# kalenforn/clip-based-cross-modal-hash

Hardware: AMD Instinct MI355X
Metric: Hamming query x gallery pairs/sec (fused mAP@all pass, DCMHT COCO-shaped 64-bit) (higher is better)
Workload: dtype u32; 1 GPU; configs[1] DCMHT COCO 64-bit retrieval: Q=5000 queries x R=117218 gallery items per GPU (x1 GPUs, contiguous shards), K=64 bits, C=80 classes, mAP@all; Q=5000, R_per_gpu=117218, K=64, C=80, parallelism=gallery-shard x1, query_blocks=1

## Files before the change

### clip-based-cross-modal-hash_amd/csrc/xmh_scan.hip

```cpp
#include "xmh_common.h"
#include <atomic>
#include <math.h>
#include <mutex>
#include <string.h>
#include <vector>
#include "xmh_scan_bits.h"
#include "xmh_scan_mfma.h"
#include "xmh_scan_kernels.h"

#include <stdlib.h>
#include <type_traits>

namespace {

constexpr int kSlotBudget64 = 9 * 1024;
constexpr int kSlotBudget32 = 5 * 1024;
constexpr int slots_for(int W, bool tern, int counter_bytes) {
    const int nbmax = (tern ? 64 : 32) * W + 1;
    const int budget = counter_bytes == 8 ? kSlotBudget64 : kSlotBudget32;
    const int cap = W > 8 ? 64 : 8;
    int S = 2;
    while (S < cap && nbmax * (64 / S) * counter_bytes > budget) S *= 2;
    return S;
}
inline int instance_words(int W) { return W <= 1 ? 1 : (W <= 2 ? 2 : (W <= 4 ? 4 : (W <= 8 ? 8 : (W <= 16 ? 16 : (W <= 32 ? 32 : 64))))); }
constexpr bool pair_cache_shape(int W, bool tern) { return !tern && (W == 1 || W == 2 || W == 4 || W == 8); }
template <int W, bool TERN>
constexpr bool kPairCacheShape = pair_cache_shape(W, TERN);
constexpr int cache_slots(int W) { return W <= 2 ? 4 : 8; }
static_assert(slots_for(2, false, 4) == 4 && slots_for(2, false, 8) == 4 && slots_for(4, false, 4) == 8 && slots_for(4, false, 8) == 8 &&
              slots_for(8, false, 4) == 8 && slots_for(8, false, 8) == 8, "33..256 bits: the cache geometry is the uncached kernels' own");
constexpr int waves_for(int W, bool tern) { return (W >= 32 && !tern) ? 8 : 1; }
inline size_t aos_ring_bytes(int W, int LW, bool tern) { return (size_t)64 * (((W * (tern ? 2 : 1) + LW) + 3) / 4 * 4) * 4; }

struct WsLayout {
    size_t chunk_hist, below, tot, dpre, cap, tick, gate, ap_part, pair_cache, total;
};

bool r2_selfcheck_ok();
inline bool mfma_env_on() {
    const char* e = getenv("XMH_SCAN_MFMA");
    return !(e && atoi(e) == 0);
}
struct Overrides {
    int mfma = -1;
    bool masked = false;
    bool describe = false;
};
enum class Family { kValu, kR2, kR2w, kBits, kTBits };
Family pass1_family(int K, bool ternary, const Overrides& ov) {
    if (ov.mfma == 0 || !mfma_env_on()) return Family::kValu;
    if (ternary) return K <= 256 ? Family::kTBits : Family::kValu;
    if (K > 128) return K <= 256 ? Family::kBits : Family::kValu;
    if (ov.mfma < 0 && !r2_selfcheck_ok()) return Family::kValu;
    return K <= 64 ? Family::kR2 : Family::kR2w;
}
inline int tbits_tiles(int K) { return K <= 64 ? 2 : (K <= 128 ? 4 : 8); }
inline int ap_r2_mode() {
    const char* e = getenv("XMH_SCAN_AP_R2");
    return e ? (atoi(e) != 0 ? 1 : 0) : 2;
}
constexpr int kAp2Waves = 4, kAp2Groups = 2;
constexpr int kMfmaWaves = 4;
static_assert(xmh::kScanBitsWaves == kMfmaWaves, "k_scan_hist_b takes the plan's query tiles of 64");
constexpr int kBitsMaxChunk = 24192;
struct R2Geom { int nw, nq, blocks_per_cu; int queries() const { return nw * nq * 16; } };
inline R2Geom r2_geom(int K) { return K <= 32 ? R2Geom{4, 4, 1} : (K <= 64 ? R2Geom{4, 4, 2} : R2Geom{4, 2, 2}); }

inline long long cache_cap_mb() {
    const char* cap_env = getenv("XMH_SCAN_CACHE_MB");
    return cap_env ? atoll(cap_env) : 131072;
}
inline bool ap_c_on() {
    const char* e = getenv("XMH_SCAN_AP_C");
    return !(e && atoi(e) == 0);
}
size_t pair_cache_bytes(const xmh_scan_plan& p, int K, bool ternary, Family f) {
    const long long cap_mb = cache_cap_mb();
    const bool tb = f == Family::kTBits;
    if ((ternary && !tb) || K > 256 || cap_mb <= 0 || (!tb && K <= 32 && f != Family::kR2)) return 0;
    if (f == Family::kR2 && ap_r2_mode() == 1) return 0;
    const int S = tb ? 8 : (K <= 64 ? 4 : 8);
    const size_t bytes = (size_t)p.nchunk * (size_t)(p.nqtile * S) * (size_t)((p.chunk + 63) / 64) * (S == 4 ? 1024 : 64 * 4 * xmh::kCache12Dwords);
    return bytes <= (size_t)cap_mb << 20 ? bytes : 0;
}

WsLayout ws_layout(const xmh_scan_plan& p, size_t cache_bytes) {
    WsLayout L;
    const size_t cells = (size_t)p.nchunk * p.nbuckets * p.qpad;
    size_t o = 0;
    auto take = [&](size_t bytes) {
        const size_t at = o;
        o += (bytes + 255) & ~(size_t)255;
        return at;
    };
    L.chunk_hist = take(cells * 4);
    L.below = take(cells * 8);
    L.tot = take((size_t)p.nbuckets * p.qpad * 8);
    L.dpre = take((size_t)p.nbuckets * p.qpad * 8);
    L.cap = take((size_t)p.qpad * 4);
    L.tick = take((size_t)p.nqtile * 4);
    L.gate = take(256 + 8 * 4096);
    L.ap_part = take((size_t)p.nchunk * p.qpad * 4);
    L.pair_cache = take(cache_bytes);
    L.total = o;
    return L;
}

size_t cache_for_workspace(const xmh_scan_plan& p, int K, bool ternary, Family f, size_t ws_bytes) {
    const size_t c = pair_cache_bytes(p, K, ternary, f);
    return c && ws_bytes < ws_layout(p, c).total ? 0 : c;
}

int make_plan(int64_t Q, int64_t R, int K, int ternary, xmh_scan_plan* p, const Overrides& ov = {}) {
    if (Q <= 0 || R <= 0 || K <= 0) return xmh::fail(XMH_EINVAL, "scan plan: bad shape Q=%lld R=%lld K=%d", (long long)Q, (long long)R, K);
    if (R >= (1ll << 24) || Q >= (1ll << 24)) return xmh::fail(XMH_ENOTSUP, "scan plan: shard too large (R=%lld, Q=%lld)", (long long)R, (long long)Q);
    const int64_t nb = ternary ? 2 * (int64_t)K + 1 : (int64_t)K + 1;
    const int Wd = (K + 31) / 32;
    if (Wd > 64 || (ternary && Wd > 8))
        return xmh::fail(XMH_ENOTSUP, "scan plan: K=%d%s (at most 2048 code bits, 256 with zero planes)", K, ternary ? " ternary" : "");
    const int S64 = slots_for(instance_words(Wd), ternary != 0, 8);
    const int64_t lds_ap = nb * (64 / S64) * 8;
    if (lds_ap > 150 * 1024) return xmh::fail(XMH_ENOTSUP, "scan plan: %lld distance buckets need %lld B of LDS per wave; K=%d%s", (long long)nb, (long long)lds_ap, K, ternary ? " ternary" : "");
    const Family fam = pass1_family(K, ternary != 0, ov);
    const bool r2 = fam == Family::kR2 || fam == Family::kR2w;
    int64_t nqt = xmh::ceil_div(Q, 64);
    const int r2q = r2_geom(K).queries();
    if (r2) {
        int64_t l = r2q;
        while (l % 64) l += r2q;
        nqt = xmh::ceil_div(nqt * 64, l) * l / 64;
    }
    const int64_t wpc = 8;
    const int64_t slots = (int64_t)xmh::device_cu_count() * wpc;
    const bool cache_shape = !ternary && K > 32 && K <= 64 && cache_cap_mb() > 0;
    const int64_t rounds = nb <= 33 ? 3 : (nb <= 65 && !cache_shape ? 2 : 1);
    int64_t nchunk = rounds * slots / nqt;
    if (S64 > 8) nchunk = nchunk * 8 / S64;
    const bool mfma = fam != Family::kValu;
    bool fill = false;
    if (mfma) {
        int64_t bsets = nb <= 129 ? 6 : 3;
        if (const char* e = xmh_experiment_env("XMH_BITS_SETS")) bsets = atoi(e) > 0 ? atoi(e) : bsets;
        nchunk = bsets * xmh::device_cu_count() / nqt;
        if (r2) {
            int sets = K > 32 && K <= 64 ? 1 : 2;
            if (const char* e = xmh_experiment_env("XMH_R2_SETS")) sets = atoi(e) > 0 ? atoi(e) : sets;
            nchunk = (int64_t)sets * xmh::device_cu_count() * r2_geom(K).blocks_per_cu / (nqt * 64 / r2q);
            if (const char* e = xmh_experiment_env("XMH_R2_FILL")) fill = atoi(e) != 0 && fam == Family::kR2 && sets == 1 && cache_shape && ap_r2_mode() != 1;
        }
    }
    if (nchunk < 1) nchunk = 1;
    if (nchunk > 8 && !fill) nchunk = (nchunk + 4) / 8 * 8;
    int64_t chunk = xmh::ceil_div(R, nchunk);
    if (chunk < kMinChunk) chunk = kMinChunk;
    if (chunk > kMaxChunk) chunk = kMaxChunk;
    chunk = xmh::ceil_div(chunk, 8) * 8;
    if (mfma) {
        chunk = xmh::ceil_div(chunk, 64) * 64;
        int64_t bits_max = kBitsMaxChunk;
        if (const char* e = xmh_experiment_env("XMH_BITS_MAX_CHUNK")) bits_max = atoll(e) / 64 * 64 > 0 ? atoll(e) / 64 * 64 : bits_max;
        if (!r2 && chunk > bits_max) {
            nchunk = xmh::ceil_div(xmh::ceil_div(R, bits_max), 8) * 8;
            chunk = xmh::ceil_div(xmh::ceil_div(R, nchunk), 64) * 64;
        }
    }
    nchunk = xmh::ceil_div(R, chunk);
    p->chunk = chunk;
    p->nchunk = nchunk;
    p->nqtile = nqt;
    p->qpad = nqt * 64;
    p->nbuckets = nb;
    p->ws_bytes = ws_layout(*p, pair_cache_bytes(*p, K, ternary != 0, fam)).total;
    return XMH_OK;
}

int lane_order_ok(hipStream_t st) {
    static int cached[64];
    static bool have[64];
    static std::mutex mu;
    int dev = 0;
    if (hipGetDevice(&dev) != hipSuccess || dev < 0 || dev >= 64) return 0;
    if (getenv("XMH_SCAN_MASKED") != nullptr) return 0;
    std::lock_guard<std::mutex> lock(mu);
    if (have[dev]) return cached[dev];
    int ok = 0;
    {
        const char* fe = getenv("XMH_SCAN_PROBE_FAULT");
        const int fault = fe && atoi(fe) != 0;
        uint32_t* flag = nullptr;
        float* sink = nullptr;
        if (hipMalloc(&flag, 8) == hipSuccess && hipMalloc(&sink, 256) == hipSuccess) {
            uint32_t h[2] = {0, 1};
            int cus = xmh::device_cu_count();
            if (hipMemsetAsync(flag, 0, 8, st) == hipSuccess) {
                hipLaunchKernelGGL(k_probe_lane_order, dim3(1), dim3(64), 0, st, flag);
                hipLaunchKernelGGL(k_probe_lane_order_load, dim3((unsigned)(cus * 25)), dim3(64), 0, st, flag + 1, fault, sink);
                if (hipGetLastError() == hipSuccess && hipMemcpyAsync(h, flag, 8, hipMemcpyDeviceToHost, st) == hipSuccess && hipStreamSynchronize(st) == hipSuccess)
                    ok = h[0] == 1u && h[1] == 0u;
            }
        }
        if (flag) (void)hipFree(flag);
        if (sink) (void)hipFree(sink);
        if (!ok)
            fprintf(stderr, "xmh: the lane-order probe FAILED on device %d%s: same-address returning LDS adds are not served in lane order here; "
                            "pass 2 runs the masked kernels (about 2x slower, same results).\n", dev, fault ? " (XMH_SCAN_PROBE_FAULT set: forced)" : "");
    }
    cached[dev] = ok;
    have[dev] = true;
    return ok;
}

struct DevBuf {
    void* p = nullptr;
    ~DevBuf() { if (p) (void)hipFree(p); }
    bool alloc(size_t n) { return hipMalloc(&p, n) == hipSuccess; }
    template <typename T> T* as() { return static_cast<T*>(p); }
};

template <bool TERN, typename F>
int dispatch_shape(int W, int LW, F&& f) {
#define XMH_CASE(WW, LL) \
    if (W == WW && LW == LL) return f(std::integral_constant<int, WW>{}, std::integral_constant<int, LL>{});
    XMH_CASE(1, 1) XMH_CASE(1, 2) XMH_CASE(1, 3) XMH_CASE(1, 4)
    XMH_CASE(2, 1) XMH_CASE(2, 2) XMH_CASE(2, 3) XMH_CASE(2, 4)
    XMH_CASE(4, 1) XMH_CASE(4, 2) XMH_CASE(4, 3) XMH_CASE(4, 4)
    XMH_CASE(8, 1) XMH_CASE(8, 2) XMH_CASE(8, 3) XMH_CASE(8, 4)
    if constexpr (!TERN) {
        XMH_CASE(1, 8) XMH_CASE(2, 8) XMH_CASE(4, 8) XMH_CASE(8, 8)
    }
    if constexpr (!TERN) {
        XMH_CASE(16, 1) XMH_CASE(16, 2) XMH_CASE(16, 3) XMH_CASE(16, 4)
        XMH_CASE(32, 1) XMH_CASE(32, 2) XMH_CASE(32, 3) XMH_CASE(32, 4)
        XMH_CASE(64, 1) XMH_CASE(64, 2) XMH_CASE(64, 3) XMH_CASE(64, 4)
    }
#undef XMH_CASE
    return xmh::fail(XMH_ENOTSUP, "scan: unsupported shape W=%d code words (K in {<=32,64,128,256}, binary also 512,1024,2048), Lw=%d label words (C<=128; binary codes up to 256 bits also exactly 8 words: 129..256 classes)%s",
                     W, LW, TERN ? ", ternary" : "");
}

int packed_rank_bits(int K, int64_t R) {
    const char* e = getenv("XMH_SCAN_PACK32");
    if (e && e[0] == '0') return 0;
    if (!(K > 64 || (e && e[0] == 'a'))) return 0;
    const int64_t rank_max = R + 2;
    int rank_bits = 0;
    while ((1ll << rank_bits) < rank_max) ++rank_bits;
    return rank_bits > 24 ? 0 : rank_bits;
}

enum class Mode { kUnsharded, kBaseAll, kTotals, kAllToAll };
struct ScanCall {
    const uint32_t *qbits, *qzero, *qlab, *rbits, *rzero, *rlab;
    int64_t Q, R; int K, C;
    void* ws; size_t ws_bytes;
    bool tern;
};
struct Pass2 {
    Mode mode; int64_t k;
    double* ap_sum; int32_t* cap;
    double* map_out;
    const uint32_t *base_all = nullptr, *base_rel = nullptr, *nrel_total = nullptr;
    const uint32_t* hist_g = nullptr;
    int world = 0, rank = 0;
};
enum class Kern { kHistS, kHistR2, kHistR2w, kHistB, kApS, kApC, kApR2 };
enum Gate : unsigned {
    kBySize = 1,
    kByWrap = 2,
    kByWidth = 4,
};
struct Launch {
    Kern kern = Kern::kHistS;
    int W = 0, LW = 0;
    bool tern = false, cache = false;
    int S = 0, NW = 1;
    int nml = 0;
    int eb = 0; bool half = false;
    bool p32 = false, masked = false;
    unsigned gate = 0;
    bool stand_in = false;
};
struct ScanRoute {
    Launch p1;
    size_t cache_bytes = 0;
    int rank_bits = 0;
    Launch p2[3];
    int n2 = 0;
};

ScanRoute scan_route(const xmh_scan_plan& p, const ScanCall& c, Mode mode, const Overrides& ov, hipStream_t st) {
    ScanRoute r;
    const int K = c.K, C = c.C; const bool tern = c.tern; const int64_t R = c.R;
    const Family fam = pass1_family(K, tern, ov);
    const int W = ov.describe ? instance_words((K + 31) / 32) : (K + 31) / 32, LW = (C + 31) / 32;
    const bool lane_ok = ov.describe || (!ov.masked && lane_order_ok(st));
    r.cache_bytes = cache_for_workspace(p, K, tern, fam, c.ws_bytes);
    const bool cache = r.cache_bytes != 0;
    const bool mfma = fam != Family::kValu && LW <= 4 && lane_ok;
    Launch& h = r.p1;
    h.W = W; h.LW = LW; h.tern = tern; h.cache = cache; h.nml = LW <= 2 ? 1 : 2;
    if (!mfma) {
        h.cache = cache && pair_cache_shape(W, tern);
        h.S = h.cache ? cache_slots(W) : slots_for(W, tern, 4);
        h.NW = h.S == 64 ? waves_for(W, tern) : 1;
    } else if (fam == Family::kBits || fam == Family::kTBits) {
        h.kern = Kern::kHistB;
        h.S = fam == Family::kTBits ? tbits_tiles(K) : 4;
    } else {
        const R2Geom g = r2_geom(K);
        h.kern = fam == Family::kR2 ? Kern::kHistR2 : Kern::kHistR2w;
        h.NW = g.nw; h.S = g.nq;
    }
    const bool sharded = mode != Mode::kUnsharded;
    const bool masked = !lane_ok;
    const int rank_bits = sharded || masked ? 0 : packed_rank_bits(K, R);
    const bool fits_fb = sharded || R <= kFloatBitsMaxItems;
    const bool apc_on = ap_c_on();
    const bool byte128 = cache && mfma && fam == Family::kR2w;
    const bool tb = cache && mfma && fam == Family::kTBits;
    const bool apc = cache && apc_on && (byte128 || (K <= 64 && rank_bits == 0)) && !tern && !masked && (mode != Mode::kBaseAll || byte128) && fits_fb;
    const bool apr2 = !cache && mfma && fam == Family::kR2 && ap_r2_mode() != 0 && !masked && mode != Mode::kBaseAll && rank_bits == 0 && fits_fb;
    const bool apc16 = cache && apc_on && ((K > 128 && K <= 256 && !tern) || tb) && !masked && !sharded && R <= kFloatBitsMaxItems;
    const unsigned size_gate = sharded && (apc || apr2) ? kBySize : 0u;
    r.rank_bits = byte128 && apc ? 0 : rank_bits;
    auto add = [&](Kern kern, unsigned gate) -> Launch& { Launch& l = r.p2[r.n2++]; l.kern = kern; l.gate = gate; return l; };
    if (apc) {
        Launch& l = add(Kern::kApC, size_gate | (byte128 ? kByWrap : 0u));
        l.eb = 8; l.half = byte128; l.S = byte128 ? 8 : 4;
    }
    if (apr2) {
        Launch& l = add(Kern::kApR2, size_gate);
        l.W = W; l.LW = LW; l.nml = h.nml; l.NW = kAp2Waves; l.S = kAp2Groups;
    }
    if (apc16) {
        Launch& l = add(Kern::kApC, kByWidth);
        l.eb = 16; l.S = 8;
    }
    if ((apc || apr2) && !size_gate && !byte128) return r;
    Launch s;
    s.kern = Kern::kApS; s.W = tb ? 8 : W; s.LW = LW; s.tern = tern && !tb; s.masked = masked;
    s.cache = cache && !byte128 && !masked && pair_cache_shape(s.W, s.tern);
    s.stand_in = byte128 && apc;
    s.gate = size_gate | (s.stand_in ? kByWrap : 0u) | (r.rank_bits ? kByWidth : 0u);
    for (const bool p32 : {true, false}) {
        if (p32 ? r.rank_bits == 0 : apc16) continue;
        s.p32 = p32;
        s.S = s.cache ? cache_slots(s.W) : slots_for(s.W, s.tern, p32 ? 4 : 8);
        s.NW = s.S == 64 ? waves_for(s.W, s.tern) : 1;
        r.p2[r.n2++] = s;
    }
    return r;
}

int describe_launch(const Launch& l, char* out, size_t n) {
    static const char* const tf[2] = {"false", "true"};
    auto exists = [&](auto tern_c) { return dispatch_shape<decltype(tern_c)::value>(l.W, l.LW, [](auto, auto) { return (int)XMH_OK; }); };
    switch (l.kern) {
    case Kern::kHistS:
    case Kern::kApS:
        if (const int rc = l.tern ? exists(std::true_type{}) : exists(std::false_type{})) return rc;
        if (l.kern == Kern::kHistS) snprintf(out, n, "k_scan_hist_s<%d, %d, %s, %d, %d, %s>", l.W, l.LW, tf[l.tern], l.S, l.NW, tf[l.cache]);
        else
            snprintf(out, n, "k_scan_ap_s<%d, %d, %s, %s, %d, %s, %s, %d, %s>", l.W, l.cache ? 1 : l.LW, tf[l.tern], tf[!l.cache], l.S, tf[l.p32], tf[l.masked],
                     l.NW, tf[l.cache]);
        break;
    case Kern::kHistR2:
    case Kern::kHistR2w:
        snprintf(out, n, "k_scan_hist_%s<%d, %d, %d, %s>", l.kern == Kern::kHistR2 ? "r2" : "r2w", l.nml, l.NW, l.S, tf[l.cache]);
        break;
    case Kern::kHistB: {
        int nsh, nqt;
        xmh::scan_hist_bits_shape(l.S, l.tern, &nsh, &nqt);
        snprintf(out, n, "k_scan_hist_b<%d, %d, %d, %d, %s, %s>", l.S, kMfmaWaves, nsh, nqt, tf[l.cache], tf[l.tern]);
        break;
    }
    case Kern::kApC: snprintf(out, n, "k_scan_ap_c<false, %d, %s>", l.eb, tf[l.half]); break;
    case Kern::kApR2: snprintf(out, n, "k_scan_ap_r2<%d, %d, %d, false>", l.nml, l.NW, l.S); break;
    }
    return XMH_OK;
}

int check_common(const char* who, const ScanCall& c, const xmh_scan_plan& p) {
    if (!c.qbits || !c.rbits || !c.qlab || !c.rlab || !c.ws) return xmh::fail(XMH_EINVAL, "%s: null pointer", who);
    if ((c.qzero == nullptr) != (c.rzero == nullptr)) return xmh::fail(XMH_EINVAL, "%s: zero masks must be given for both sides or neither", who);
    if (c.C <= 0) return xmh::fail(XMH_EINVAL, "%s: C=%d", who, c.C);
    const size_t need = ws_layout(p, 0).total;
    if (c.ws_bytes < need) return xmh::fail(XMH_EINVAL, "%s: workspace too small (%zu < %zu; %zu with the pair cache)", who, c.ws_bytes, need, (size_t)p.ws_bytes);
    return XMH_OK;
}

ScanArgs make_args(const ScanCall& c, const xmh_scan_plan& p) {
    return ScanArgs{c.qbits, c.qzero, c.qlab, c.rbits, c.rzero, c.rlab, (int)c.Q, (int)c.R, c.K, (int)p.chunk, (int)p.nchunk, (int)p.nqtile, (int)p.qpad,
                    (int)p.nbuckets, nullptr, (int)p.nqtile};
}

MfmaArgs r2_args(const ScanCall& c, const Launch& l, const xmh_scan_plan& p, int nqt) {
    MfmaArgs a{c.qbits, (int)c.Q, (int)c.R, c.K, l.W, (int)p.chunk, (int)p.nchunk, nqt, (int)p.nbuckets, (int)p.qpad};
    a.rbits = c.rbits; a.rlab = c.rlab; a.qlab = c.qlab; a.LW = l.LW;
    return a;
}

struct Geom { unsigned grid, block; size_t lds; int nqt, nrun; };
Geom launch_geom(const Launch& l, const xmh_scan_plan& p, int64_t Q) {
    const size_t nb = (size_t)p.nbuckets;
    const bool ap = l.kern == Kern::kApS || l.kern == Kern::kApC || l.kern == Kern::kApR2;
    Geom g{0, 64u * (unsigned)l.NW, 0, 0};
    if (l.kern == Kern::kHistS || l.kern == Kern::kApS) {
        g.lds = ((nb * (64 / l.S) * (ap && !l.p32 ? 2 : 1) + 3) & ~(size_t)3) * 4 * l.NW + (ap && l.cache ? 0 : aos_ring_bytes(l.W, l.LW, l.tern));
        g.nqt = (int)p.nqtile * l.S / l.NW;
    } else if (l.kern == Kern::kApC) {
        g.lds = nb * (64 / l.S) * 8; g.nqt = (int)p.nqtile * l.S;
    } else if (l.kern == Kern::kHistB) {
        g.nqt = (int)(p.qpad / (16 * kMfmaWaves));
    } else {
        g.lds = (size_t)l.NW * l.S * nb * 16 * (ap ? 8 : 4); g.nqt = (int)(p.qpad / (l.NW * l.S * 16));
    }
    g.nrun = g.nqt;
    if (ap) {
        static const bool all_tiles = xmh_experiment_env("XMH_AP_TILES") && atoi(xmh_experiment_env("XMH_AP_TILES")) == 0;
        if (!all_tiles) g.nrun = (int)xmh::ceil_div(Q, p.qpad / g.nqt);
    }
    g.grid = xmh::scan_grid_blocks(g.nrun, (int)p.nchunk);
    return g;
}

template <typename KernT, typename... Args>
int start(const char* who, const Launch& l, const Geom& g, hipStream_t st, KernT kern, int S, int NW, bool cache, Args... args) {
    if (l.S != S || l.NW != NW || l.cache != cache)
        return xmh::fail(XMH_ENOTSUP, "%s: the route names an instance with S=%d NW=%d cache=%d, the one compiled for W=%d LW=%d has S=%d NW=%d cache=%d", who, l.S,
                         l.NW, (int)l.cache, l.W, l.LW, S, NW, (int)cache);
    if (const int rc = xmh::raise_dynamic_lds(reinterpret_cast<const void*>(kern), g.lds, who)) return rc;
    hipLaunchKernelGGL(kern, dim3(g.grid), dim3(g.block), g.lds, st, args...);
    return XMH_OK;
}

struct ScanCtx {
    const ScanCall& c;
    hipStream_t st;
    xmh_scan_plan p;
    ScanRoute r;
    WsLayout L;
    ScanArgs a;
    uint32_t kcap = 0xffffffffu;
    bool capped = false;
    template <typename T> T* at(size_t off) const { return reinterpret_cast<T*>(static_cast<char*>(c.ws) + off); }
    uint32_t* chunk_hist() const { return at<uint32_t>(L.chunk_hist); }
    const uint2* below() const { return at<uint2>(L.below); }
    uint2* tot() const { return at<uint2>(L.tot); }
    uint2* dpre() const { return at<uint2>(L.dpre); }
    uint32_t* cap_ws() const { return at<uint32_t>(L.cap); }
    float* ap_part() const { return at<float>(L.ap_part); }
    ScanArgs args(const Geom& g, bool cached) const { ScanArgs as = a; as.nqt = g.nqt; as.nrun = g.nrun; as.pair_cache = cached ? pair_cache() : nullptr; return as; }
    uint32_t* gate(int word = 0) const { return at<uint32_t>(L.gate) + word; }
    const uint32_t* gate_if(const Launch& l, unsigned g, int word) const { return (l.gate & g) ? gate(word) : nullptr; }
    uint4* pair_cache() const { return r.cache_bytes ? at<uint4>(L.pair_cache) : nullptr; }
};

int plan_call(const char* who, ScanCtx& x, const Overrides& ov) {
    if (const int rc = make_plan(x.c.Q, x.c.R, x.c.K, x.c.tern, &x.p, ov)) return rc;
    return check_common(who, x.c, x.p);
}
void route_call(ScanCtx& x, Mode mode, const Overrides& ov) {
    x.r = scan_route(x.p, x.c, mode, ov, x.st);
    x.a = make_args(x.c, x.p);
    x.L = ws_layout(x.p, x.r.cache_bytes);
}

int valu_hist(const ScanCtx& x) {
    const Launch& h = x.r.p1;
    const Geom g = launch_geom(h, x.p, x.c.Q);
    const ScanArgs as = x.args(g, h.cache);
    auto go = [&](auto kern, int S, int NW, bool cache) {
        xmh::ProfScope prof("scan_hist", x.st);
        return start("xmh_hamming_hist", h, g, x.st, kern, S, NW, cache, as, x.chunk_hist());
    };
    auto launch = [&](auto tern_c) {
        constexpr bool T = decltype(tern_c)::value;
        return dispatch_shape<T>(h.W, h.LW, [&](auto w, auto l) {
            constexpr int WW = decltype(w)::value, LL = decltype(l)::value;
            if constexpr (kPairCacheShape<WW, T>) {
                if (h.cache) return go(k_scan_hist_s<WW, LL, T, cache_slots(WW), 1, true>, cache_slots(WW), 1, true);
            }
            constexpr int S = slots_for(WW, T, 4);
            constexpr int NW = S == 64 ? waves_for(WW, T) : 1;
            return go(k_scan_hist_s<WW, LL, T, S, NW, false>, S, NW, false);
        });
    };
    return h.tern ? launch(std::true_type{}) : launch(std::false_type{});
}

int mfma_hist(const ScanCtx& x) {
    const Launch& h = x.r.p1;
    const xmh_scan_plan& p = x.p;
    const Geom g = launch_geom(h, p, x.c.Q);
    uint32_t* chunk_hist = x.chunk_hist();
    uint4* cache = x.pair_cache();
    if (h.kern == Kern::kHistB) {
        xmh::ScanBitsArgs a{x.c.rbits, x.c.rlab, x.c.qbits, x.c.qlab, (int)x.c.Q, (int)x.c.R, x.c.K, h.W, h.LW, (int)p.chunk, (int)p.nchunk, g.nqt,
                            (int)p.nbuckets, (int)p.qpad};
        a.rzero = x.c.rzero; a.qzero = x.c.qzero;
        return xmh::launch_scan_hist_bits(a, h.S, chunk_hist, cache, x.st);
    }
    hipLaunchKernelGGL(k_scan_touch, dim3(xmh::scan_grid_blocks(kTouchPerChunk, (int)p.nchunk)), dim3(256), 0, x.st, x.c.rbits, x.c.rlab, x.c.R, h.W, h.LW,
                       p.chunk, (int)p.nchunk, x.at<uint32_t>(x.L.tick), (int)((x.L.gate + 256 - x.L.tick) / 4));
    XMH_LAUNCH_CHECK("xmh_hamming_hist control words");
    const MfmaArgs a = r2_args(x.c, h, p, g.nqt);
    xmh::ProfScope prof("scan_hist", x.st);
    auto go = [&](auto kern, int NW, int NQ, bool cached, auto... wrap_word) { return start("xmh_hamming_hist", h, g, x.st, kern, NQ, NW, cached, a, chunk_hist, cache, wrap_word...); };
    if (h.kern == Kern::kHistR2w) {
        uint32_t* ovf = x.gate(kGateWrapped);
        return h.nml == 1 ? (h.cache ? go(k_scan_hist_r2w<1, 4, 2, true>, 4, 2, true, ovf) : go(k_scan_hist_r2w<1, 4, 2, false>, 4, 2, false, ovf))
                          : (h.cache ? go(k_scan_hist_r2w<2, 4, 2, true>, 4, 2, true, ovf) : go(k_scan_hist_r2w<2, 4, 2, false>, 4, 2, false, ovf));
    }
    return h.nml == 1 ? (h.cache ? go(k_scan_hist_r2<1, 4, 4, true>, 4, 4, true) : go(k_scan_hist_r2<1, 4, 4, false>, 4, 4, false))
                      : (h.cache ? go(k_scan_hist_r2<2, 4, 4, true>, 4, 4, true) : go(k_scan_hist_r2<2, 4, 4, false>, 4, 4, false));
}

int hamming_hist_impl(const ScanCall& c, uint32_t* hist_all, uint32_t* hist_rel, xmh_stream_t stream, const Overrides& ov) {
    ScanCtx x{c, xmh::as_stream(stream)};
    if (const int rc = plan_call("xmh_hamming_hist", x, ov)) return rc;
    route_call(x, Mode::kUnsharded, ov);
    const xmh_scan_plan& p = x.p;
    const Kern kern = x.r.p1.kern;
    if (kern == Kern::kHistS || kern == Kern::kHistB) XMH_HIP(hipMemsetAsync(x.at<char>(x.L.tick), 0, x.L.gate + 256 - x.L.tick, x.st));
    if (const int rc = kern == Kern::kHistS ? valu_hist(x) : mfma_hist(x)) return rc;
    XMH_LAUNCH_CHECK("xmh_hamming_hist");
    hipLaunchKernelGGL(k_scan_below, dim3((unsigned)p.nqtile, (unsigned)xmh::ceil_div(p.nbuckets, 4)), dim3(256), 0, x.st, x.chunk_hist(), (int)p.qpad,
                       (int)p.nbuckets, (int)p.nchunk, kern != Kern::kHistS ? kRelHi16 : 0u, x.at<uint2>(x.L.below), x.tot(), x.at<uint32_t>(x.L.tick), (int)c.Q, x.dpre(),
                       x.cap_ws(), x.gate(), hist_all, hist_rel);
    XMH_LAUNCH_CHECK("xmh_hamming_hist below");
    return XMH_OK;
}

}

extern "C" int xmh_scan_plan_make(int64_t Q, int64_t R, int K, int ternary, xmh_scan_plan* plan_host) {
    if (!plan_host) return xmh::fail(XMH_EINVAL, "xmh_scan_plan_make: null plan");
    return make_plan(Q, R, K, ternary, plan_host);
}

extern "C" size_t xmh_scan_pair_cache_bytes(int64_t Q, int64_t R, int K, int ternary) {
    xmh_scan_plan p;
    if (make_plan(Q, R, K, ternary, &p)) return 0;
    return pair_cache_bytes(p, K, ternary != 0, pass1_family(K, ternary != 0, {}));
}

extern "C" size_t xmh_scan_pair_cache_offset(int64_t Q, int64_t R, int K, int ternary) {
    xmh_scan_plan p;
    if (make_plan(Q, R, K, ternary, &p)) return (size_t)-1;
    return ws_layout(p, 0).pair_cache;
}

extern "C" size_t xmh_scan_ws_bytes_nocache(int64_t Q, int64_t R, int K, int ternary) {
    xmh_scan_plan p;
    if (make_plan(Q, R, K, ternary, &p)) return 0;
    return ws_layout(p, 0).total;
}

extern "C" int xmh_scan_describe(int64_t Q, int64_t R, int K, int C, int ternary, char* out, size_t out_bytes) {
    if (!out || out_bytes < 64) return xmh::fail(XMH_EINVAL, "xmh_scan_describe: buffer too small");
    xmh_scan_plan p;
    if (const int rc = make_plan(Q, R, K, ternary, &p)) return rc;
    Overrides ov;
    ov.describe = true;
    const ScanCall c{nullptr, nullptr, nullptr, nullptr, nullptr, nullptr, Q, R, K, C, nullptr, (size_t)p.ws_bytes, ternary != 0};
    const ScanRoute r = scan_route(p, c, Mode::kUnsharded, ov, nullptr);
    char p1[160], p2[200] = "", one[120];
    if (const int rc = describe_launch(r.p1, p1, sizeof(p1))) return rc;
    for (const bool p32 : {true, false})
        for (int i = 0; i < r.n2; ++i) {
            if (r.p2[i].stand_in || r.p2[i].p32 != p32) continue;
            if (const int rc = describe_launch(r.p2[i], one, sizeof(one))) return rc;
            const size_t at = strlen(p2);
            snprintf(p2 + at, sizeof(p2) - at, "%s%s", at ? "|" : "", one);
        }
    if ((size_t)snprintf(out, out_bytes, "pass1=%s;pass2=%s", p1, p2) >= out_bytes) return xmh::fail(XMH_EINVAL, "xmh_scan_describe: buffer too small");
    return XMH_OK;
}

extern "C" int xmh_hamming_hist(const uint32_t* qbits, const uint32_t* qzero, const uint32_t* qlab,
                                const uint32_t* rbits, const uint32_t* rzero, const uint32_t* rlab, int64_t Q, int64_t R,
                                int K, int C, void* ws, size_t ws_bytes, uint32_t* hist_all, uint32_t* hist_rel,
                                xmh_stream_t stream) {
    XMH_RANGE("xmh_hamming_hist (pass 1)");
    const ScanCall c{qbits, qzero, qlab, rbits, rzero, rlab, Q, R, K, C, ws, ws_bytes, qzero != nullptr};
    return hamming_hist_impl(c, hist_all, hist_rel, stream, {});
}

namespace {
int ap_offsets(const ScanCtx& x, const Pass2& o) {
    const xmh_scan_plan& p = x.p;
    if (o.mode == Mode::kUnsharded) return XMH_OK;
    if (o.mode == Mode::kAllToAll)
        hipLaunchKernelGGL(k_shard_scatter_offsets, dim3((unsigned)xmh::ceil_div(p.qpad, 256), (unsigned)p.nbuckets + 1), dim3(256), 0, x.st,
                           reinterpret_cast<const uint2*>(o.hist_g), (int)p.nbuckets, (int)(p.qpad / o.world), (int)x.c.Q, (int)p.qpad, o.k, x.dpre(), x.cap_ws(),
                           o.cap, x.gate(2));
    else if (o.mode == Mode::kTotals)
        hipLaunchKernelGGL(k_shard_offsets_dpre, dim3((unsigned)p.nqtile), dim3(256), 0, x.st, reinterpret_cast<const uint2*>(o.hist_g), o.world, o.rank,
                           (int)x.c.Q, (int)p.qpad, (int)p.nbuckets, o.k, x.dpre(), x.cap_ws(), o.cap, x.gate(2));
    else
        hipLaunchKernelGGL(k_scan_dpre, dim3((unsigned)p.nqtile), dim3(256), 0, x.st, (const uint2*)x.tot(), (int)x.c.Q, (int)p.qpad, (int)p.nbuckets, o.base_all,
                           o.base_rel, o.nrel_total, o.k, x.dpre(), x.cap_ws(), o.cap, (uint32_t*)nullptr, (uint32_t*)nullptr, (uint32_t*)nullptr, x.gate(2));
    XMH_LAUNCH_CHECK(o.mode == Mode::kAllToAll ? "xmh_hamming_map_sharded_offsets scatter" : (o.mode == Mode::kTotals ? "xmh_hamming_map_sharded offsets" : "xmh_hamming_ap dpre"));
    return XMH_OK;
}

int ap_launch_c(const ScanCtx& x, const Launch& l) {
    const Geom g = launch_geom(l, x.p, x.c.Q);
    const ScanArgs as = x.args(g, true);
    xmh::ProfScope prof("scan_ap", x.st);
    auto go = [&](auto kc, int S) {
        return start("xmh_hamming_ap", l, g, x.st, kc, S, 1, l.cache, as, x.below(), (const uint2*)x.dpre(), (const uint32_t*)x.cap_ws(), x.ap_part(),
                     x.gate_if(l, kBySize, 2), x.kcap, x.gate_if(l, kByWrap, kGateWrapped), x.gate_if(l, kByWidth, 0), l.gate & kByWidth ? x.r.rank_bits : 0);
    };
    if (l.eb == 16) return x.capped ? go(k_scan_ap_c<true, 16>, 8) : go(k_scan_ap_c<false, 16>, 8);
    if (l.half) return x.capped ? go(k_scan_ap_c<true, 8, true>, 8) : go(k_scan_ap_c<false, 8, true>, 8);
    return x.capped ? go(k_scan_ap_c<true, 8>, 4) : go(k_scan_ap_c<false, 8>, 4);
}

int ap_launch_r2(const ScanCtx& x, const Launch& l) {
    const Geom g = launch_geom(l, x.p, x.c.Q);
    const MfmaArgs ma = r2_args(x.c, l, x.p, g.nrun);
    xmh::ProfScope prof("scan_ap", x.st);
    auto go = [&](auto kern) {
        return start("xmh_hamming_ap", l, g, x.st, kern, kAp2Groups, kAp2Waves, l.cache, ma, x.below(), (const uint2*)x.dpre(), (const uint32_t*)x.cap_ws(), x.ap_part(),
                     x.gate_if(l, kBySize, 2), x.kcap);
    };
    return l.nml == 1 ? (x.capped ? go(k_scan_ap_r2<1, kAp2Waves, kAp2Groups, true>) : go(k_scan_ap_r2<1, kAp2Waves, kAp2Groups, false>))
                      : (x.capped ? go(k_scan_ap_r2<2, kAp2Waves, kAp2Groups, true>) : go(k_scan_ap_r2<2, kAp2Waves, kAp2Groups, false>));
}

int ap_launch_s(const ScanCtx& x, const Launch& l) {
    const Geom g = launch_geom(l, x.p, x.c.Q);
    const ScanArgs as = x.args(g, l.cache);
    auto go = [&](auto kern, int S, int NW, bool cache, const uint32_t* run_if) {
        xmh::ProfScope prof(l.p32 ? "scan_ap32" : "scan_ap", x.st);
        return start("xmh_hamming_ap", l, g, x.st, kern, S, NW, cache, as, x.below(), (const uint2*)x.dpre(), (const uint32_t*)x.cap_ws(), x.ap_part(),
                     (const uint32_t*)x.gate(), x.r.rank_bits, x.kcap, x.gate_if(l, kBySize, 2), run_if);
    };
    auto by_shape = [&](auto tern_c, auto cap_c, auto p32_c, auto masked_c) {
        constexpr bool T = decltype(tern_c)::value, CP = decltype(cap_c)::value, P32 = decltype(p32_c)::value, MK = decltype(masked_c)::value;
        return dispatch_shape<T>(l.W, l.LW, [&](auto w, auto lw) {
            constexpr int WW = decltype(w)::value, LL = decltype(lw)::value;
            if constexpr (P32 && MK) return xmh::fail(XMH_ENOTSUP, "xmh_hamming_ap: the masked fallback runs 64-bit counters only");
            else {
                if constexpr (kPairCacheShape<WW, T> && !MK) {
                    if (l.cache)
                        return go(k_scan_ap_s<WW, 1, T, CP, cache_slots(WW), P32, MK, 1, true>, cache_slots(WW), 1, true, nullptr);
                }
                (void)CP;
                constexpr int S = slots_for(WW, T, P32 ? 4 : 8);
                constexpr int NW = S == 64 ? waves_for(WW, T) : 1;
                return go(k_scan_ap_s<WW, LL, T, true, S, P32, MK, NW, false>, S, NW, false, x.gate_if(l, kByWrap, kGateWrapped));
            }
        });
    };
    using T1 = std::true_type; using T0 = std::false_type;
    auto by_mask = [&](auto t, auto c, auto w) { return l.masked ? by_shape(t, c, w, T1{}) : by_shape(t, c, w, T0{}); };
    auto by_width = [&](auto t, auto c) { return l.p32 ? by_mask(t, c, T1{}) : by_mask(t, c, T0{}); };
    auto by_cap = [&](auto t) { return x.capped ? by_width(t, T1{}) : by_width(t, T0{}); };
    return l.tern ? by_cap(T1{}) : by_cap(T0{});
}

int ap_reduce(const ScanCtx& x, const Pass2& o) {
    const int64_t Q = x.c.Q;
    const unsigned nred = (unsigned)xmh::ceil_div(Q, 64);
    if (o.map_out && nred <= 4096) {
        hipLaunchKernelGGL(k_ap_reduce_map, dim3(nred), dim3(256), 0, x.st, (const float*)x.ap_part(), (int)Q, (int)x.p.qpad, (int)x.p.nchunk,
                           (const uint32_t*)x.cap_ws(), x.kcap, o.cap, o.ap_sum, x.at<double>(x.L.gate + 256), x.gate(1), o.map_out);
        XMH_LAUNCH_CHECK("xmh_hamming_map reduce+finalize");
        return XMH_OK;
    }
    hipLaunchKernelGGL(k_ap_reduce, dim3(nred), dim3(256), 0, x.st, (const float*)x.ap_part(), (int)Q, (int)x.p.qpad, (int)x.p.nchunk, o.ap_sum,
                       o.mode != Mode::kUnsharded ? (const uint32_t*)nullptr : (const uint32_t*)x.cap_ws(), x.kcap, o.cap);
    XMH_LAUNCH_CHECK("xmh_hamming_ap reduce");
    if (o.map_out) {
        hipLaunchKernelGGL(k_map_finalize, dim3(1), dim3(256), 0, x.st, (const double*)o.ap_sum, (const int32_t*)o.cap, Q, o.map_out);
        XMH_LAUNCH_CHECK("xmh_hamming_map finalize");
    }
    return XMH_OK;
}

static std::atomic<int> g_verify{0};
constexpr int XMH_EVERIFY_CODE = -74;

int hamming_ap_impl(const ScanCall& c, const Pass2& o, xmh_stream_t stream, const Overrides& ov);

int verify_against_masked(const ScanCall& c, const Pass2& o, xmh_stream_t stream) {
    hipStream_t st = xmh::as_stream(stream);
    const int64_t Q = c.Q;
    std::vector<double> a1((size_t)Q), a0((size_t)Q);
    std::vector<int32_t> c1((size_t)Q), c0((size_t)Q);
    XMH_HIP(hipMemcpyAsync(a1.data(), o.ap_sum, (size_t)Q * 8, hipMemcpyDeviceToHost, st));
    XMH_HIP(hipMemcpyAsync(c1.data(), o.cap, (size_t)Q * 4, hipMemcpyDeviceToHost, st));
    XMH_HIP(hipStreamSynchronize(st));
    Overrides ov;
    ov.mfma = 0;
    ov.masked = true;
    xmh_scan_plan p;
    if (const int rc = make_plan(Q, c.R, c.K, c.tern, &p, ov)) return rc;
    const size_t small = ws_layout(p, 0).total;
    DevBuf ws2, ap2, cap2;
    if (!ws2.alloc(small) || !ap2.alloc((size_t)Q * 8) || !cap2.alloc((size_t)Q * 4))
        return xmh::fail(XMH_ENOMEM, "xmh_scan_verify: no room for the second evaluation (%zu bytes)", small);
    ScanCall again = c; again.ws = ws2.p; again.ws_bytes = small;
    const Pass2 o2{Mode::kUnsharded, o.k, ap2.as<double>(), cap2.as<int32_t>(), nullptr};
    if (const int rc = hamming_hist_impl(again, nullptr, nullptr, stream, ov)) return rc;
    if (const int rc = hamming_ap_impl(again, o2, stream, ov)) return rc;
    XMH_HIP(hipMemcpyAsync(a0.data(), ap2.p, (size_t)Q * 8, hipMemcpyDeviceToHost, st));
    XMH_HIP(hipMemcpyAsync(c0.data(), cap2.p, (size_t)Q * 4, hipMemcpyDeviceToHost, st));
    XMH_HIP(hipStreamSynchronize(st));
    if (const char* fe = getenv("XMH_SCAN_VERIFY_FAULT")) {
        const int64_t at = atoll(fe) % Q;
        a1[(size_t)at] *= 1.0 + 1e-3;
    }
    int64_t bad = -1, nbad = 0;
    for (int64_t i = 0; i < Q; ++i) {
        const bool same = c1[(size_t)i] == c0[(size_t)i] && fabs(a1[(size_t)i] - a0[(size_t)i]) <= 4e-6 * fabs(a0[(size_t)i]) + 1e-9;
        if (!same) { if (bad < 0) bad = i; ++nbad; }
    }
    if (nbad)
        return xmh::fail(XMH_EVERIFY_CODE, "xmh_scan_verify: %lld of %lld queries differ between the lane-order kernels and the masked re-derivation "
                         "(first: query %lld, AP sum %.9g vs %.9g, divisor %d vs %d)", (long long)nbad, (long long)Q, (long long)bad, a1[(size_t)bad], a0[(size_t)bad],
                         c1[(size_t)bad], c0[(size_t)bad]);
    return XMH_OK;
}

int hamming_ap_impl(const ScanCall& c, const Pass2& o, xmh_stream_t stream, const Overrides& ov) {
    ScanCtx x{c, xmh::as_stream(stream)};
    if (const int rc = plan_call("xmh_hamming_ap", x, ov)) return rc;
    if (!o.ap_sum || !o.cap) return xmh::fail(XMH_EINVAL, "xmh_hamming_ap: null output");
    const int ext = (o.base_all != nullptr) + (o.base_rel != nullptr) + (o.nrel_total != nullptr);
    if (ext != 0 && ext != 3) return xmh::fail(XMH_EINVAL, "xmh_hamming_ap: base_all, base_rel and nrel_total go together");
    route_call(x, o.mode, ov);
    x.kcap = o.k > 0 && o.k < (int64_t)0xffffffffll ? (uint32_t)o.k : 0xffffffffu;
    x.capped = o.k > 0;
    if (const int rc = ap_offsets(x, o)) return rc;
    for (int i = 0; i < x.r.n2; ++i) {
        const Launch& l = x.r.p2[i];
        if (const int rc = l.kern == Kern::kApC ? ap_launch_c(x, l) : (l.kern == Kern::kApR2 ? ap_launch_r2(x, l) : ap_launch_s(x, l))) return rc;
        XMH_LAUNCH_CHECK("xmh_hamming_ap");
    }
    if (const int rc = ap_reduce(x, o)) return rc;
    if (g_verify.load(std::memory_order_relaxed) && !ov.masked && o.mode == Mode::kUnsharded) return verify_against_masked(c, o, stream);
    return XMH_OK;
}

bool selfcheck_eval(const ScanCall& c, int force, std::vector<uint32_t>& hist, std::vector<double>& ap, std::vector<int32_t>& cap) {
    Overrides ov;
    ov.mfma = force;
    const int64_t Q = c.Q;
    xmh_scan_plan p;
    if (make_plan(Q, c.R, c.K, 0, &p, ov) != XMH_OK) return false;
    const size_t nb = (size_t)p.nbuckets;
    DevBuf ws, dh, dap, dcap;
    if (!ws.alloc(p.ws_bytes) || !dh.alloc(2 * Q * nb * 4) || !dap.alloc(Q * 8) || !dcap.alloc(Q * 4)) return false;
    ScanCall run = c; run.ws = ws.p; run.ws_bytes = p.ws_bytes;
    const Pass2 o{Mode::kUnsharded, 0, dap.as<double>(), dcap.as<int32_t>(), nullptr};
    uint32_t* h = dh.as<uint32_t>();
    if (hamming_hist_impl(run, h, h + Q * nb, nullptr, ov) != XMH_OK) return false;
    if (hamming_ap_impl(run, o, nullptr, ov) != XMH_OK) return false;
    hist.resize(2 * Q * nb); ap.resize(Q); cap.resize(Q);
    if (hipDeviceSynchronize() != hipSuccess) return false;
    return hipMemcpy(hist.data(), dh.p, hist.size() * 4, hipMemcpyDeviceToHost) == hipSuccess && hipMemcpy(ap.data(), dap.p, Q * 8, hipMemcpyDeviceToHost) == hipSuccess &&
           hipMemcpy(cap.data(), dcap.p, Q * 4, hipMemcpyDeviceToHost) == hipSuccess;
}

bool r2_selfcheck_ok() {
    static int state[64];
    static std::mutex mu;
    int dev = 0;
    if (hipGetDevice(&dev) != hipSuccess || dev < 0 || dev >= 64) return true;
    const char* e = getenv("XMH_SCAN_M2_SELFCHECK");
    if (e && atoi(e) == 0) return true;
    std::lock_guard<std::mutex> lock(mu);
    if (state[dev]) return state[dev] == 1;
    state[dev] = 1;
    const int64_t Q = 200, R = 9000;
    bool same = true, ran = true;
    const int cases[6][2] = {{64, 80}, {40, 80}, {16, 80}, {100, 80}, {64, 128}, {100, 128}};
    for (const auto& kc : cases) {
        const int K = kc[0], C = kc[1], LW = (C + 31) / 32;
        const int W = (K + 31) / 32;
        std::vector<uint32_t> qb(Q * W), ql(Q * LW), rb(R * W), rl(R * LW);
        uint64_t x = 0x9E3779B97F4A7C15ull ^ (uint64_t)K;
        auto rnd = [&]() { x ^= x << 13; x ^= x >> 7; x ^= x << 17; return (uint32_t)(x >> 16); };
        const uint32_t last = K % 32 ? (1u << (K % 32)) - 1 : 0xffffffffu;
        for (auto& v : qb) v = rnd();
        for (int64_t i = 0; i < R; ++i)
            for (int w = 0; w < W; ++w) rb[i * W + w] = (i > 64 && (rnd() & 3) == 0) ? rb[(rnd() % 64) * W + w] : rnd();
        for (int64_t i = 0; i < Q; ++i) qb[i * W + W - 1] &= last;
        for (int64_t i = 0; i < R; ++i) rb[i * W + W - 1] &= last;
        const uint32_t lastl = C % 32 ? (1u << (C % 32)) - 1 : 0xffffffffu;
        for (int64_t i = 0; i < Q * LW; ++i) ql[i] = rnd() & rnd() & rnd() & (i % LW == LW - 1 ? lastl : 0xffffffffu);
        for (int64_t i = 0; i < R * LW; ++i) rl[i] = rnd() & rnd() & rnd() & (i % LW == LW - 1 ? lastl : 0xffffffffu);
        if (C == 80) {
            for (int64_t i = 0; i < Q; ++i) ql[i * LW] |= 1u;
            for (int64_t i = 0; i < R; i += 7) rl[i * LW] |= 1u;
        } else {
            auto one = [&](uint32_t* l, int c) { for (int w = 0; w < LW; ++w) l[w] = 0u; l[c >> 5] = 1u << (c & 31); };
            for (int64_t i = 0; i < Q; i += 2) one(&ql[i * LW], i % 8 == 0 ? (int)(i * 3 % 64) : 64 + (int)(i * 7 % 64));
            for (int64_t i = 0; i < R; ++i) {
                if (i % 3 == 0) one(&rl[i * LW], 64 + (int)(i * 5 % 64));
                else if (i % 3 == 1) for (int w = 0; w < LW; ++w) rl[i * LW + w] = 0u;
            }
            for (int w = 0; w < LW; ++w) ql[1 * LW + w] = rl[2 * LW + w] = rl[5000 * LW + w] = 0xffffffffu;
        }
        std::vector<uint32_t> h1, h0;
        std::vector<double> a1, a0;
        std::vector<int32_t> c1, c0;
        DevBuf dq, dql, dr, drl;
        auto up = [](DevBuf& d, const std::vector<uint32_t>& v) { return d.alloc(v.size() * 4) && hipMemcpy(d.p, v.data(), v.size() * 4, hipMemcpyHostToDevice) == hipSuccess; };
        if (!up(dq, qb) || !up(dql, ql) || !up(dr, rb) || !up(drl, rl)) { ran = false; break; }
        const ScanCall c{dq.as<uint32_t>(), nullptr, dql.as<uint32_t>(), dr.as<uint32_t>(), nullptr, drl.as<uint32_t>(), Q, R, K, C, nullptr, 0, false};
        if (!selfcheck_eval(c, 1, h1, a1, c1) || !selfcheck_eval(c, 0, h0, a0, c0)) { ran = false; break; }
        bool ap_close = true;
        for (int64_t i = 0; i < Q; ++i) ap_close = ap_close && fabs(a1[i] - a0[i]) <= 4e-6 * fabs(a0[i]) + 1e-9;
        if (h1 != h0 || c1 != c0 || !ap_close) { same = false; break; }
    }
    if (e && atoi(e) == 2) same = false;
    if (!ran) {
        state[dev] = 0;
        return true;
    }
    if (!same) {
        state[dev] = 2;
        fprintf(stderr, "xmh: k_scan_hist_r2 self-check FAILED on device %d (results differ from the VALU kernels): falling back to the VALU scan "
                        "for this process.  Please report the hipcc / ROCm versions.\n", dev);
    }
    return state[dev] == 1;
}
}

extern "C" int xmh_scan_verify(int on) {
    g_verify.store(on != 0 ? 1 : 0, std::memory_order_relaxed);
    return XMH_OK;
}

extern "C" int xmh_hamming_ap(const uint32_t* qbits, const uint32_t* qzero, const uint32_t* qlab, const uint32_t* rbits,
                              const uint32_t* rzero, const uint32_t* rlab, int64_t Q, int64_t R, int K, int C, void* ws,
                              size_t ws_bytes, const uint32_t* base_all, const uint32_t* base_rel,
                              const uint32_t* nrel_total, int64_t k, double* ap_sum, int32_t* cap, xmh_stream_t stream) {
    XMH_RANGE("xmh_hamming_ap (pass 2)");
    const ScanCall c{qbits, qzero, qlab, rbits, rzero, rlab, Q, R, K, C, ws, ws_bytes, qzero != nullptr};
    Pass2 o{base_all ? Mode::kBaseAll : Mode::kUnsharded, k, ap_sum, cap, nullptr};
    o.base_all = base_all; o.base_rel = base_rel; o.nrel_total = nrel_total;
    return hamming_ap_impl(c, o, stream, {});
}

extern "C" int xmh_hamming_map(const uint32_t* qbits, const uint32_t* qzero, const uint32_t* qlab, const uint32_t* rbits,
                               const uint32_t* rzero, const uint32_t* rlab, int64_t Q, int64_t R, int K, int C, void* ws,
                               size_t ws_bytes, int64_t k, double* ap_sum, int32_t* cap, double* map_out, xmh_stream_t stream) {
    XMH_RANGE("xmh_hamming_map (pass 2 + mean)");
    if (!map_out) return xmh::fail(XMH_EINVAL, "xmh_hamming_map: null output");
    const ScanCall c{qbits, qzero, qlab, rbits, rzero, rlab, Q, R, K, C, ws, ws_bytes, qzero != nullptr};
    return hamming_ap_impl(c, Pass2{Mode::kUnsharded, k, ap_sum, cap, map_out}, stream, {});
}

extern "C" size_t xmh_scan_totals_offset(int64_t Q, int64_t R, int K, int ternary, size_t* bytes) {
    xmh_scan_plan p;
    if (make_plan(Q, R, K, ternary, &p)) return (size_t)-1;
    if (bytes) *bytes = (size_t)p.nbuckets * p.qpad * 8;
    return ws_layout(p, 0).tot;
}

extern "C" int xmh_hamming_map_sharded(const uint32_t* qbits, const uint32_t* qzero, const uint32_t* qlab, const uint32_t* rbits,
                                       const uint32_t* rzero, const uint32_t* rlab, int64_t Q, int64_t R, int K, int C, void* ws,
                                       size_t ws_bytes, const uint32_t* hist_gathered, int world, int rank, int64_t k, double* ap_sum,
                                       int32_t* cap, double* map_partial, xmh_stream_t stream) {
    XMH_RANGE("xmh_hamming_map_sharded (pass 2)");
    if (!hist_gathered || !map_partial) return xmh::fail(XMH_EINVAL, "xmh_hamming_map_sharded: null pointer");
    if (world <= 0 || rank < 0 || rank >= world) return xmh::fail(XMH_EINVAL, "xmh_hamming_map_sharded: bad world=%d rank=%d", world, rank);
    const ScanCall c{qbits, qzero, qlab, rbits, rzero, rlab, Q, R, K, C, ws, ws_bytes, qzero != nullptr};
    Pass2 o{Mode::kTotals, k, ap_sum, cap, map_partial};
    o.hist_g = hist_gathered; o.world = world; o.rank = rank;
    return hamming_ap_impl(c, o, stream, {});
}

extern "C" int xmh_shard_slice_offsets(const uint32_t* totals_slices, int world, int nbuckets, int slice, uint32_t* offsets_out, xmh_stream_t stream) {
    XMH_RANGE("xmh_shard_slice_offsets");
    if (!totals_slices || !offsets_out) return xmh::fail(XMH_EINVAL, "xmh_shard_slice_offsets: null pointer");
    if (world <= 0 || nbuckets <= 0 || slice <= 0) return xmh::fail(XMH_EINVAL, "xmh_shard_slice_offsets: bad arguments (world=%d nb=%d slice=%d)", world, nbuckets, slice);
    hipLaunchKernelGGL(k_shard_slice_offsets, dim3((unsigned)xmh::ceil_div(slice, 64)), dim3(256), 0, xmh::as_stream(stream),
                       reinterpret_cast<const uint2*>(totals_slices), world, nbuckets, slice, reinterpret_cast<uint2*>(offsets_out));
    XMH_LAUNCH_CHECK("xmh_shard_slice_offsets");
    return XMH_OK;
}

extern "C" int xmh_hamming_map_sharded_offsets(const uint32_t* qbits, const uint32_t* qzero, const uint32_t* qlab, const uint32_t* rbits,
                                               const uint32_t* rzero, const uint32_t* rlab, int64_t Q, int64_t R, int K, int C, void* ws,
                                               size_t ws_bytes, const uint32_t* offsets, int world, int64_t k, double* ap_sum, int32_t* cap,
                                               double* map_partial, xmh_stream_t stream) {
    XMH_RANGE("xmh_hamming_map_sharded_offsets (pass 2)");
    if (!offsets || !map_partial) return xmh::fail(XMH_EINVAL, "xmh_hamming_map_sharded_offsets: null pointer");
    const ScanCall c{qbits, qzero, qlab, rbits, rzero, rlab, Q, R, K, C, ws, ws_bytes, qzero != nullptr};
    xmh_scan_plan p;
    if (const int rc = make_plan(Q, R, K, c.tern, &p)) return rc;
    if (world <= 0 || p.qpad % world) return xmh::fail(XMH_EINVAL, "xmh_hamming_map_sharded_offsets: qpad=%lld is not a multiple of world=%d", (long long)p.qpad, world);
    Pass2 o{Mode::kAllToAll, k, ap_sum, cap, map_partial};
    o.hist_g = offsets; o.world = world;
    return hamming_ap_impl(c, o, stream, {});
}

extern "C" int xmh_map_finalize(const double* ap_sum, const int32_t* cap, int64_t Q, double* map_out, xmh_stream_t stream) {
    XMH_RANGE("xmh_map_finalize");
    if (!ap_sum || !cap || !map_out || Q <= 0) return xmh::fail(XMH_EINVAL, "xmh_map_finalize: bad arguments");
    hipLaunchKernelGGL(k_map_finalize, dim3(1), dim3(256), 0, xmh::as_stream(stream), ap_sum, cap, Q, map_out);
    XMH_LAUNCH_CHECK("xmh_map_finalize");
    return XMH_OK;
}

extern "C" int xmh_shard_offsets(const uint32_t* hist_gathered, int world, int rank, int64_t Q, int nbuckets, uint32_t* base_all,
                                 uint32_t* base_rel, uint32_t* nrel_total, xmh_stream_t stream) {
    XMH_RANGE("xmh_shard_offsets");
    if (!hist_gathered || !base_all || !base_rel || !nrel_total) return xmh::fail(XMH_EINVAL, "xmh_shard_offsets: null pointer");
    if (world <= 0 || rank < 0 || rank >= world || Q <= 0 || nbuckets <= 0 || Q >= (1ll << 24))
        return xmh::fail(XMH_EINVAL, "xmh_shard_offsets: bad arguments (world=%d rank=%d Q=%lld nb=%d)", world, rank, (long long)Q, nbuckets);
    hipLaunchKernelGGL(k_shard_offsets, dim3((unsigned)Q), dim3(64), 0, xmh::as_stream(stream), hist_gathered, world, rank, (int)Q, nbuckets,
                       base_all, base_rel, nrel_total);
    XMH_LAUNCH_CHECK("xmh_shard_offsets");
    return XMH_OK;
}
```

### clip-based-cross-modal-hash_amd/csrc/xmh_scan_mfma.h

```cpp
#pragma once
#include "xmh_common.h"
#include "xmh_scan_map.h"
#include <type_traits>

namespace {

constexpr int kMaxChunk = 32768;
constexpr uint32_t kF23 = 0x4B000000u;
constexpr int64_t kFloatBitsMaxItems = (1ll << 23) - 3;
constexpr int kMinChunk = 256;

struct ScanArgs {
    const uint32_t* qbits;
    const uint32_t* qzero;
    const uint32_t* qlab;
    const uint32_t* rbits;
    const uint32_t* rzero;
    const uint32_t* rlab;
    int Q, R, K;
    int chunk, nchunk, nqt, qpad, nb;
    uint4* pair_cache;
    int nrun;
};

__device__ __forceinline__ bool map_block(const ScanArgs& a, int& chunk_id, int& qtile) {
    return xmh::scan_block_map((int)blockIdx.x, a.nrun, a.nchunk, chunk_id, qtile);
}

typedef int v4i __attribute__((ext_vector_type(4)));

struct MfmaArgs {
    const uint32_t* qbits;
    int Q, R, K, W;
    int chunk, nchunk, nqt, nb, qpad;
    const uint32_t* rbits = nullptr;
    const uint32_t* rlab = nullptr;
    const uint32_t* qlab = nullptr;
    int LW = 0;
};

__device__ __forceinline__ bool map_block(const MfmaArgs& a, int& chunk_id, int& qtile) {
    return xmh::scan_block_map((int)blockIdx.x, a.nqt, a.nchunk, chunk_id, qtile);
}

__device__ __forceinline__ v4i label_query_f4(uint32_t w, uint32_t one) {
    v4i r;
#pragma unroll
    for (int j = 0; j < 4; ++j) r[j] = (int)(((w >> j) & 0x11111111u) * one);
    return r;
}
__device__ __forceinline__ v4i label_item_f4(uint32_t w) {
    return v4i{(int)(w & 0x11111111u), (int)(w & 0x22222222u), (int)(w & 0x44444444u), (int)((w >> 1) & 0x44444444u)};
}

template <int NML, int NW, int NQ, bool CACHE>
__device__ __forceinline__ void scan_hist_r2_body(const MfmaArgs& a, uint32_t* __restrict__ chunk_hist, uint4* __restrict__ pair_cache) {
    static_assert(NML == 1 || NML == 2, "one i8 label tile (at most 64 classes) or one FP4 label tile (65-128 classes)");
    constexpr bool F4 = NML == 2;
    constexpr int NMI = 2, NMQ = 3;
    constexpr bool REGS = true;
    extern __shared__ __attribute__((aligned(16))) uint32_t lds[];
    int chunk_id, qtile;
    if (!map_block(a, chunk_id, qtile)) return;
    const int lane = threadIdx.x & 63, wave = threadIdx.x >> 6;
    const int ql = lane & 15, slot = lane >> 4;
    const int t16 = (qtile * NW + wave) * NQ;
    const int ncell = a.nb * 16;
    uint32_t* cnt = lds + (wave * NQ) * ncell;
    for (int e = lane; e < NQ * ncell; e += 64) cnt[e] = 0u;
    v4i bq[NQ][NMQ], cq[NQ], kqv[REGS ? NQ : 1];
    bool valid[NQ];
    const int rsh = 4 * (slot & 1), rwi = slot >> 1;
#pragma unroll
    for (int h = 0; h < NQ; ++h) {
        valid[h] = (t16 + h) * 16 + ql < a.Q;
        int pcq = 0;
        {
            const int64_t q = (int64_t)(t16 + h) * 16 + ql;
            uint32_t qw = 0u;
            if (valid[h]) {
                for (int w = 0; w < a.W; ++w) pcq += __popc(a.qbits[q * a.W + w]);
                if (rwi < a.W) qw = a.qbits[q * a.W + rwi];
            }
            qw >>= rsh;
#pragma unroll
            for (int j = 0; j < 4; ++j) {
                const uint32_t t = (qw >> j) & 0x01010101u;
                const bool on = valid[h] && rwi < a.W;
                if (j & 1) {
                    bq[h][0][j] = on ? (int)(0x20202020u ^ (t * 0xc0u)) : 0;
                    bq[h][1][j] = on ? (int)(0x01010101u ^ (t * 0xfeu)) : 0;
                } else {
                    bq[h][0][j] = on ? (int)(0x40404040u ^ (t << 7)) : 0;
                    bq[h][1][j] = on ? (int)(0x02020202u ^ (t * 0xfcu)) : 0;
                }
            }
            if constexpr (F4) {
                bq[h][2] = label_query_f4(valid[h] && slot < a.LW ? a.qlab[q * a.LW + slot] : 0u, 0x2u);
            } else {
                uint32_t lw = 0u;
                if (valid[h] && rwi < a.LW) lw = a.qlab[q * a.LW + rwi];
                lw >>= rsh;
#pragma unroll
                for (int j = 0; j < 4; ++j) bq[h][2][j] = (int)((lw >> j) & 0x01010101u);
            }
            const int k2 = 2 * pcq;
            kqv[h] = v4i{k2, k2, k2, k2};
        }
        const int c0 = (int)(uint32_t)(uintptr_t)(__attribute__((address_space(3))) uint32_t*)(cnt + h * ncell) + ql * 4 + (valid[h] ? 64 * pcq : 0);
        cq[h] = v4i{c0, c0, c0, c0};
    }
    v4i lab0 = {0x10000, 0x10000, 0x10000, 0x10000};
    asm volatile("" : "+v"(lab0));
#pragma unroll
    for (int h = 0; h < NQ; ++h) asm volatile("" : "+v"(cq[h]));
#pragma unroll
    for (int h = 0; h < (REGS ? NQ : 1); ++h) asm volatile("" : "+v"(kqv[h]));
    const int64_t lo = (int64_t)chunk_id * a.chunk;
    const int64_t hi = (lo + a.chunk < a.R) ? lo + a.chunk : a.R;
    const int nbat = (int)((hi - lo + 63) >> 6);
    const int64_t bat0 = lo >> 6;
    uint4* crow[NQ];
#pragma unroll
    for (int h = 0; h < NQ; ++h)
        crow[h] = CACHE ? pair_cache + ((int64_t)chunk_id * (a.qpad >> 4) + (t16 + h)) * ((a.chunk + 63) >> 6) * 64 + lane : nullptr;
    uint32_t wcur[4][NMI], wnxt[4][NMI];
    const int ritem = 4 * (lane & 3) + ((lane & 15) >> 2);
    const int wi_c = rwi < a.W ? rwi : a.W - 1;
    const int lwi = F4 ? slot : rwi;
    const int wi_l = lwi < a.LW ? lwi : (a.LW > 0 ? a.LW - 1 : 0);
    auto load_words = [&](int64_t batch, uint32_t (&w)[4][NMI]) {
        const int64_t first = batch * 64;
        if (first + 64 <= (int64_t)a.R) {
            const uint32_t* __restrict__ pc = a.rbits + (first + ritem) * a.W + wi_c;
            const uint32_t* __restrict__ pl = a.rlab + (first + ritem) * a.LW + wi_l;
#pragma unroll
            for (int g = 0; g < 4; ++g) {
                w[g][0] = pc[g * 16 * a.W];
                w[g][1] = pl[g * 16 * a.LW];
            }
        } else {
#pragma unroll
            for (int g = 0; g < 4; ++g) {
                const int64_t item = first + g * 16 + ritem;
                const int64_t it = item < a.R ? item : (int64_t)a.R - 1;
                const uint32_t ok = item < a.R ? 0xffffffffu : 0u;
                w[g][0] = a.rbits[it * a.W + wi_c] & ok;
                w[g][1] = a.rlab[it * a.LW + wi_l] & ok;
            }
        }
    };
    auto build = [&](v4i (&At)[NMI], const uint32_t (&w)[NMI]) {
        const uint32_t xa = w[0] >> rsh, xb = w[0] >> (rsh + 2);
        At[0][0] = (int)(xa & 0x01010101u);
        At[0][1] = (int)(xa & 0x02020202u);
        At[0][2] = (int)(xb & 0x01010101u);
        At[0][3] = (int)(xb & 0x02020202u);
        if constexpr (F4) {
            At[1] = label_item_f4(w[1]);
        } else {
            const uint32_t y = w[1] >> rsh;
#pragma unroll
            for (int j = 0; j < 4; ++j) At[1][j] = (int)(y & (0x01010101u << j));
        }
    };
    load_words(bat0, wcur);
#ifdef XMH_ABL_NOBUILD
    v4i A[4][NMI];
#endif
    for (int i = 0; i < nbat; ++i) {
#ifdef XMH_ABL_NOLOADW
        if (i == 0) load_words(bat0, wnxt);
#else
        load_words(bat0 + (i + 1 < nbat ? i + 1 : i), wnxt);
#endif
#ifndef XMH_ABL_NOBUILD
        v4i A[REGS ? 4 : 2][NMI];
#endif
        uint32_t cw[NQ][4];
        v4i addr_p, d2_p, lab_p;
#ifndef XMH_R2_NOPS
#define XMH_R2_NOPS 0
#endif
#if XMH_R2_NOPS == 0
#define XMH_R2_OPEN "s_nop 3\n\t"
#define XMH_R2_EVAL_CLOSE "s_nop 7"
#define XMH_R2_TAIL "s_nop 7\n\ts_nop 3"
#elif XMH_R2_NOPS == 1
#define XMH_R2_OPEN "s_nop 1\n\t"
#define XMH_R2_EVAL_CLOSE "s_nop 7"
#define XMH_R2_TAIL "s_nop 7\n\ts_nop 3"
#elif XMH_R2_NOPS == 2
#define XMH_R2_OPEN ""
#define XMH_R2_EVAL_CLOSE "s_nop 7"
#define XMH_R2_TAIL "s_nop 7\n\ts_nop 3"
#elif XMH_R2_NOPS == 3
#define XMH_R2_OPEN "s_nop 1\n\t"
#define XMH_R2_EVAL_CLOSE "s_nop 3"
#define XMH_R2_TAIL "s_nop 1"
#else
#define XMH_R2_OPEN ""
#define XMH_R2_EVAL_CLOSE "s_nop 3"
#define XMH_R2_TAIL "s_nop 1"
#endif
#ifdef XMH_ABL_NOMIN
#define XMH_VMIN "; "
#else
#define XMH_VMIN "v_min_u32 "
#endif
#ifdef XMH_ABL_MINFULL
#undef XMH_VMIN
#define XMH_VMIN "v_and_b32 "
#endif
#ifdef XMH_ABL_NOADD
#define XMH_ADD(A, D) "s_nop 0\n\t"
#else
#define XMH_ADD(A, D) "ds_add_u32 " A ", " D "\n\t"
#endif
#ifdef XMH_ABL_NOMFMA
#define XMH_MFMA(D, A, B, C) "s_nop 0\n\t"
#define XMH_MFMA_F4(D, A, B, C) "s_nop 0\n\t"
#else
#define XMH_MFMA(D, A, B, C) "v_mfma_i32_16x16x64_i8 " D ", " A ", " B ", " C "\n\t"
#define XMH_MFMA_F4(D, A, B, C) "v_mfma_f32_16x16x128_f8f6f4 " D ", " A ", " B ", " C " cbsz:4 blgp:4\n\t"
#endif
#define XMH_SDWA(J) "dst_sel:BYTE_" #J " dst_unused:UNUSED_PRESERVE src0_sel:BYTE_0 src1_sel:BYTE_0\n\t"
#define XMH_R2_FUSED_CACHE(LAB)                                                                                                                   \
    asm volatile(XMH_R2_OPEN LAB("%0", "%8", "%9", "%10")                                                                                         \
                 XMH_VMIN "%4, 0x10001, %24\n\t" XMH_VMIN "%5, 0x10001, %25\n\t" XMH_VMIN "%6, 0x10001, %26\n\t" XMH_VMIN "%7, 0x10001, %27\n\t" \
                 "v_or_b32_sdwa %3, %16, %4 dst_sel:BYTE_0 dst_unused:UNUSED_PAD src0_sel:BYTE_0 src1_sel:BYTE_0\n\t"                            \
                 XMH_ADD("%20", "%4")                                                                                                             \
                 XMH_MFMA("%1", "%11", "%12", "%13")                                                                                              \
                 "v_or_b32_sdwa %3, %17, %5 " XMH_SDWA(1) XMH_ADD("%21", "%5") "v_or_b32_sdwa %3, %18, %6 " XMH_SDWA(2)                           \
                 XMH_MFMA("%2", "%11", "%14", "%15")                                                                                              \
                 XMH_ADD("%22", "%6") "v_or_b32_sdwa %3, %19, %7 " XMH_SDWA(3) XMH_ADD("%23", "%7")                                               \
                 : "=&v"(lab), "=&v"(addr), "=&v"(d2), "=&v"(w), "=&v"(i0), "=&v"(i1), "=&v"(i2), "=&v"(i3)                                        \
                 : "v"(At[1]), "v"(bq[h][2]), "v"(lab0), "v"(At[0]), "v"(bq[h][0]), "v"(cq[h]), "v"(bq[h][1]), "v"(kqv[REGS ? h : 0]),             \
                   "v"(d2_p[0]), "v"(d2_p[1]), "v"(d2_p[2]), "v"(d2_p[3]), "v"(addr_p[0]), "v"(addr_p[1]), "v"(addr_p[2]), "v"(addr_p[3]),         \
                   "v"(lab_p[0]), "v"(lab_p[1]), "v"(lab_p[2]), "v"(lab_p[3])                                                                      \
                 : "memory")
#define XMH_R2_FUSED_PLAIN(LAB)                                                                                                                   \
    asm volatile(XMH_R2_OPEN LAB("%0", "%6", "%7", "%8")                                                                                          \
                 XMH_VMIN "%2, 0x10001, %16\n\t" XMH_VMIN "%3, 0x10001, %17\n\t" XMH_VMIN "%4, 0x10001, %18\n\t" XMH_VMIN "%5, 0x10001, %19\n\t" \
                 XMH_MFMA("%1", "%9", "%10", "%11")                                                                                               \
                 XMH_ADD("%12", "%2") XMH_ADD("%13", "%3") XMH_ADD("%14", "%4") XMH_ADD("%15", "%5")                                              \
                 : "=&v"(lab), "=&v"(addr), "=&v"(i0), "=&v"(i1), "=&v"(i2), "=&v"(i3)                                                             \
                 : "v"(At[1]), "v"(bq[h][2]), "v"(lab0), "v"(At[0]), "v"(bq[h][0]), "v"(cq[h]),                                                    \
                   "v"(addr_p[0]), "v"(addr_p[1]), "v"(addr_p[2]), "v"(addr_p[3]), "v"(lab_p[0]), "v"(lab_p[1]), "v"(lab_p[2]), "v"(lab_p[3])      \
                 : "memory")
#define XMH_R2_EVAL_CACHE(LAB)                                                                                                                    \
    asm volatile(XMH_R2_OPEN LAB("%0", "%3", "%4", "%5") XMH_MFMA("%1", "%6", "%7", "%8") XMH_MFMA("%2", "%6", "%9", "%10") XMH_R2_EVAL_CLOSE     \
                 : "=&v"(lab), "=&v"(addr), "=&v"(d2)                                                                                             \
                 : "v"(At[1]), "v"(bq[h][2]), "v"(lab0), "v"(At[0]), "v"(bq[h][0]), "v"(cq[h]), "v"(bq[h][1]), "v"(kqv[REGS ? h : 0]))
#define XMH_R2_EVAL_PLAIN(LAB)                                                                                                                    \
    asm volatile(XMH_R2_OPEN LAB("%0", "%2", "%3", "%4") XMH_MFMA("%1", "%5", "%6", "%7") XMH_R2_EVAL_CLOSE                                       \
                 : "=&v"(lab), "=&v"(addr)                                                                                                        \
                 : "v"(At[1]), "v"(bq[h][2]), "v"(lab0), "v"(At[0]), "v"(bq[h][0]), "v"(cq[h]))
        auto fused = [&](const v4i (&At)[NMI], int h, v4i& addr, v4i& d2, v4i& lab, uint32_t& w) {
            uint32_t i0, i1, i2, i3;
            if constexpr (F4 && CACHE) XMH_R2_FUSED_CACHE(XMH_MFMA_F4);
            else if constexpr (F4) XMH_R2_FUSED_PLAIN(XMH_MFMA_F4);
            else if constexpr (CACHE) XMH_R2_FUSED_CACHE(XMH_MFMA);
            else XMH_R2_FUSED_PLAIN(XMH_MFMA);
        };
        auto evaluate = [&](const v4i (&At)[NMI], int h, v4i& addr, v4i& d2, v4i& lab) {
            if constexpr (F4 && CACHE) XMH_R2_EVAL_CACHE(XMH_MFMA_F4);
            else if constexpr (F4) XMH_R2_EVAL_PLAIN(XMH_MFMA_F4);
            else if constexpr (CACHE) XMH_R2_EVAL_CACHE(XMH_MFMA);
            else XMH_R2_EVAL_PLAIN(XMH_MFMA);
        };
        auto consume = [&](uint32_t& w, const v4i (&live)[NMI]) {
            uint32_t i0, i1, i2, i3;
            if (CACHE) {
                asm volatile(
                    XMH_VMIN "%1, 0x10001, %5\n\t" XMH_VMIN "%2, 0x10001, %6\n\t" XMH_VMIN "%3, 0x10001, %7\n\t" XMH_VMIN "%4, 0x10001, %8\n\t"
                    "v_or_b32_sdwa %0, %9, %1 dst_sel:BYTE_0 dst_unused:UNUSED_PAD src0_sel:BYTE_0 src1_sel:BYTE_0\n\t"
                    XMH_ADD("%13", "%1")
                    "v_or_b32_sdwa %0, %10, %2 " XMH_SDWA(1) XMH_ADD("%14", "%2") "v_or_b32_sdwa %0, %11, %3 " XMH_SDWA(2)
                    XMH_ADD("%15", "%3") "v_or_b32_sdwa %0, %12, %4 " XMH_SDWA(3) XMH_ADD("%16", "%4")
                    : "=&v"(w), "=&v"(i0), "=&v"(i1), "=&v"(i2), "=&v"(i3)
                    : "v"(lab_p[0]), "v"(lab_p[1]), "v"(lab_p[2]), "v"(lab_p[3]), "v"(d2_p[0]), "v"(d2_p[1]), "v"(d2_p[2]), "v"(d2_p[3]), "v"(addr_p[0]),
                      "v"(addr_p[1]), "v"(addr_p[2]), "v"(addr_p[3]), "v"(live[0]), "v"(live[1]), "v"(live[NMI - 1])
                    : "memory");
            } else {
                asm volatile(
                    XMH_VMIN "%0, 0x10001, %4\n\t" XMH_VMIN "%1, 0x10001, %5\n\t" XMH_VMIN "%2, 0x10001, %6\n\t" XMH_VMIN "%3, 0x10001, %7\n\t"
                    XMH_ADD("%8", "%0") XMH_ADD("%9", "%1") XMH_ADD("%10", "%2") XMH_ADD("%11", "%3")
                    : "=&v"(i0), "=&v"(i1), "=&v"(i2), "=&v"(i3)
                    : "v"(lab_p[0]), "v"(lab_p[1]), "v"(lab_p[2]), "v"(lab_p[3]), "v"(addr_p[0]), "v"(addr_p[1]), "v"(addr_p[2]), "v"(addr_p[3]), "v"(live[0]),
                      "v"(live[1]), "v"(live[NMI - 1])
                    : "memory");
            }
        };
#undef XMH_R2_EVAL_PLAIN
#undef XMH_R2_EVAL_CACHE
#undef XMH_R2_FUSED_PLAIN
#undef XMH_R2_FUSED_CACHE
#undef XMH_SDWA
#undef XMH_ADD
#undef XMH_MFMA_F4
#undef XMH_MFMA
        auto group = [&](auto gc) {
            constexpr int G = decltype(gc)::value;
            constexpr int SET = REGS ? G : (G & 1);
#pragma unroll
            for (int h = 0; h < NQ; ++h) {
                v4i addr, d2, lab;
                if (G == 0 && h == 0) evaluate(A[SET], h, addr, d2, lab);
                else fused(A[SET], h, addr, d2, lab, cw[(h + NQ - 1) % NQ][h == 0 ? G - 1 : G]);
                addr_p = addr; d2_p = d2; lab_p = lab;
                if (REGS && G > 0 && h == 0) {
                    if constexpr (NMI == 2) asm volatile("" ::"v"(A[REGS ? G - 1 : 0][0]), "v"(A[REGS ? G - 1 : 0][1]));
                    else asm volatile("" ::"v"(A[REGS ? G - 1 : 0][0]), "v"(A[REGS ? G - 1 : 0][1]), "v"(A[REGS ? G - 1 : 0][NMI - 1]));
                }
            }
        };
#ifdef XMH_ABL_NOBUILD
        if (i == 0) {
#endif
        build(A[0], wcur[0]);
        build(A[1], wcur[1]);
        build(A[2], wcur[2]);
        build(A[3], wcur[3]);
#ifdef XMH_ABL_NOBUILD
        }
#endif
        group(std::integral_constant<int, 0>{});
        group(std::integral_constant<int, 1>{});
        group(std::integral_constant<int, 2>{});
        group(std::integral_constant<int, 3>{});
        asm volatile(XMH_R2_TAIL ::: "memory");
        consume(cw[NQ - 1][3], A[3]);
#ifdef XMH_ABL_NOSTORE
        if (CACHE && a.Q < 0) {
#else
        if (CACHE) {
#endif
#pragma unroll
            for (int h = 0; h < NQ; ++h) {
                uint4* dst = crow[h] + (int64_t)i * 64;
                __builtin_nontemporal_store(cw[h][0], &dst->x);
                __builtin_nontemporal_store(cw[h][1], &dst->y);
                __builtin_nontemporal_store(cw[h][2], &dst->z);
                __builtin_nontemporal_store(cw[h][3], &dst->w);
            }
        }
#pragma unroll
        for (int g = 0; g < 4; ++g)
#pragma unroll
            for (int m = 0; m < NMI; ++m) wcur[g][m] = wnxt[g][m];
    }
    const int npad = nbat * 64 - (int)(hi - lo);
    asm volatile("s_waitcnt lgkmcnt(0)" ::: "memory");
    if (npad > 0 && slot == 0) {
#pragma unroll
        for (int h = 0; h < NQ; ++h) {
            if (!valid[h]) continue;
            const int64_t q = (int64_t)(t16 + h) * 16 + ql;
            int dpad = 0;
            for (int w = 0; w < a.W; ++w) dpad += __popc(a.qbits[q * a.W + w]);
            cnt[h * ncell + dpad * 16 + ql] -= (uint32_t)npad << 16;
        }
    }
#pragma unroll
    for (int h = 0; h < NQ; ++h) {
        uint32_t* __restrict__ out = chunk_hist + ((int64_t)chunk_id * a.nb) * a.qpad + (t16 + h) * 16;
        for (int e = lane; e < ncell; e += 64) out[(int64_t)(e >> 4) * a.qpad + (e & 15)] = cnt[h * ncell + e];
    }
}

constexpr int kTouchPerChunk = 8;
__global__ __launch_bounds__(256) void k_scan_touch(const uint32_t* __restrict__ rbits, const uint32_t* __restrict__ rlab, int64_t R, int W, int LW, int64_t chunk,
                                                    int nchunk, uint32_t* __restrict__ ctl, int ctl_words) {
    if (blockIdx.x == 0)
        for (int e = threadIdx.x; e < ctl_words; e += 256) ctl[e] = 0u;
    int c, sub;
    if (!xmh::scan_block_map((int)blockIdx.x, kTouchPerChunk, nchunk, c, sub)) return;
    const int parts = c < (nchunk & ~7) ? kTouchPerChunk : 1;
    if (parts == 1) sub = 0;
    const int64_t lo = (int64_t)c * chunk, hi = lo + chunk < R ? lo + chunk : R;
    uint32_t acc = 0u;
    auto sweep = [&](const uint32_t* base, int64_t w0, int64_t w1) {
        for (int64_t w = w0 + ((int64_t)sub * 256 + threadIdx.x) * 32; w < w1; w += (int64_t)parts * 256 * 32) acc ^= base[w];
    };
    sweep(rbits, lo * W, hi * W);
    sweep(rlab, lo * LW, hi * LW);
    asm volatile("" ::"v"(acc));
}

#ifndef XMH_R2_ATTR
#define XMH_R2_ATTR
#endif
template <int NML, int NW, int NQ, bool CACHE>
__global__ __launch_bounds__(64 * NW) XMH_R2_ATTR void k_scan_hist_r2(MfmaArgs a, uint32_t* __restrict__ chunk_hist, uint4* __restrict__ pair_cache) {
    scan_hist_r2_body<NML, NW, NQ, CACHE>(a, chunk_hist, pair_cache);
}

#define XMH_W_MFMA(D, A, B, C) "v_mfma_i32_16x16x64_i8 %[" D "], %[" A "], %[" B "], %[" C "]\n\t"
#define XMH_W_MFMA_F4(D, A, B, C) "v_mfma_f32_16x16x128_f8f6f4 %[" D "], %[" A "], %[" B "], %[" C "] cbsz:4 blgp:4\n\t"
#define XMH_W_MIN(I, L) "v_min_u32 %[" I "], 0x10001, %[" L "]\n\t"
#define XMH_W_ADD(A, D) "ds_add_u32 %[" A "], %[" D "]\n\t"
#define XMH_W_FUSED_CACHE(LAB) \
    asm volatile("s_nop 3\n\t" LAB("lab", "al0", "bl0", "lab0") XMH_W_MIN("i0", "lp0") XMH_W_MIN("i1", "lp1") XMH_W_MIN("i2", "lp2")                \
                 XMH_W_MIN("i3", "lp3") XMH_W_ADD("ap0", "i0") XMH_W_MFMA("addr", "a0", "ba0", "cq") XMH_W_ADD("ap1", "i1")                         \
                 XMH_W_MFMA("addr", "a1", "ba1", "addr") XMH_W_ADD("ap2", "i2") XMH_W_MFMA("d2", "a0", "bd0", "kq") XMH_W_ADD("ap3", "i3")          \
                 XMH_W_MFMA("d2", "a1", "bd1", "d2")                                                                                                \
                 : [lab] "=&v"(lab), [addr] "=&v"(addr), [d2] "=&v"(d2), [i0] "=&v"(i0), [i1] "=&v"(i1), [i2] "=&v"(i2), [i3] "=&v"(i3)             \
                 : [a0] "v"(At[0]), [a1] "v"(At[1]), [al0] "v"(At[2]), [ba0] "v"(bA[h][0]), [ba1] "v"(bA[h][1]), [bd0] "v"(bD[h][0]),               \
                   [bd1] "v"(bD[h][1]), [bl0] "v"(bL[h]), [lab0] "v"(lab0), [cq] "v"(cq[h]), [kq] "v"(kq[h]), [lp0] "v"(lab_p[0]),                  \
                   [lp1] "v"(lab_p[1]), [lp2] "v"(lab_p[2]), [lp3] "v"(lab_p[3]), [ap0] "v"(addr_p[0]), [ap1] "v"(addr_p[1]), [ap2] "v"(addr_p[2]), \
                   [ap3] "v"(addr_p[3])                                                                                                             \
                 : "memory")
#define XMH_W_FUSED_PLAIN(LAB) \
    asm volatile("s_nop 3\n\t" LAB("lab", "al0", "bl0", "lab0") XMH_W_MIN("i0", "lp0") XMH_W_MIN("i1", "lp1") XMH_W_MIN("i2", "lp2")                 \
                 XMH_W_MIN("i3", "lp3") XMH_W_ADD("ap0", "i0") XMH_W_ADD("ap1", "i1") XMH_W_MFMA("addr", "a0", "ba0", "cq") XMH_W_ADD("ap2", "i2")   \
                 XMH_W_ADD("ap3", "i3") XMH_W_MFMA("addr", "a1", "ba1", "addr")                                                                      \
                 : [lab] "=&v"(lab), [addr] "=&v"(addr), [i0] "=&v"(i0), [i1] "=&v"(i1), [i2] "=&v"(i2), [i3] "=&v"(i3)                              \
                 : [a0] "v"(At[0]), [a1] "v"(At[1]), [al0] "v"(At[2]), [ba0] "v"(bA[h][0]), [ba1] "v"(bA[h][1]), [bl0] "v"(bL[h]), [lab0] "v"(lab0), \
                   [cq] "v"(cq[h]), [lp0] "v"(lab_p[0]), [lp1] "v"(lab_p[1]), [lp2] "v"(lab_p[2]), [lp3] "v"(lab_p[3]), [ap0] "v"(addr_p[0]),        \
                   [ap1] "v"(addr_p[1]), [ap2] "v"(addr_p[2]), [ap3] "v"(addr_p[3])                                                                  \
                 : "memory")
template <int NML, int NW, int NQ, bool CACHE>
__global__ __launch_bounds__(64 * NW) void k_scan_hist_r2w(MfmaArgs a, uint32_t* __restrict__ chunk_hist, uint4* __restrict__ pair_cache,
                                                           uint32_t* __restrict__ ovf) {
    static_assert(NML == 1 || NML == 2, "one i8 label tile (at most 64 classes) or one FP4 label tile (65-128 classes)");
    constexpr bool F4 = NML == 2;
    constexpr int NMC = 2, NMI = NMC + 1;
    extern __shared__ __attribute__((aligned(16))) uint32_t lds[];
    int chunk_id, qtile;
    if (!map_block(a, chunk_id, qtile)) return;
    const int lane = threadIdx.x & 63, wave = threadIdx.x >> 6;
    const int ql = lane & 15, slot = lane >> 4;
    const int t16 = (qtile * NW + wave) * NQ;
    const int ncell = a.nb * 16;
    uint32_t* cnt = lds + (wave * NQ) * ncell;
    for (int e = lane; e < NQ * ncell; e += 64) cnt[e] = 0u;
    const int rsh = 4 * (slot & 1), rwi = slot >> 1;
    v4i bA[NQ][NMC], bD[NQ][NMC], bL[NQ], cq[NQ], kq[NQ];
    bool valid[NQ];
#pragma unroll
    for (int h = 0; h < NQ; ++h) {
        const int64_t q = (int64_t)(t16 + h) * 16 + ql;
        valid[h] = q < a.Q;
        int pcq = 0;
        if (valid[h])
            for (int w = 0; w < a.W; ++w) pcq += __popc(a.qbits[q * a.W + w]);
#pragma unroll
        for (int c = 0; c < NMC; ++c) {
            const int wi = 2 * c + rwi;
            const bool on = valid[h] && wi < a.W;
            const uint32_t qw = (on ? a.qbits[q * a.W + wi] : 0u) >> rsh;
#pragma unroll
            for (int j = 0; j < 4; ++j) {
                const uint32_t t = (qw >> j) & 0x01010101u;
                if (j & 1) {
                    bA[h][c][j] = on ? (int)(0x20202020u ^ (t * 0xc0u)) : 0;
                    bD[h][c][j] = on ? (int)(0x01010101u ^ (t * 0xfeu)) : 0;
                } else {
                    bA[h][c][j] = on ? (int)(0x40404040u ^ (t << 7)) : 0;
                    bD[h][c][j] = on ? (int)(0x02020202u ^ (t * 0xfcu)) : 0;
                }
            }
        }
        if constexpr (F4) {
            bL[h] = label_query_f4(valid[h] && slot < a.LW ? a.qlab[q * a.LW + slot] : 0u, 0x2u);
        } else {
            uint32_t lw = 0u;
            if (valid[h] && rwi < a.LW) lw = a.qlab[q * a.LW + rwi];
            lw >>= rsh;
#pragma unroll
            for (int j = 0; j < 4; ++j) bL[h][j] = (int)((lw >> j) & 0x01010101u);
        }
        const int c0 = (int)(uint32_t)(uintptr_t)(__attribute__((address_space(3))) uint32_t*)(cnt + h * ncell) + ql * 4 + (valid[h] ? 64 * pcq : 0);
        const int k2 = valid[h] ? 2 * pcq : 0;
        cq[h] = v4i{c0, c0, c0, c0};
        kq[h] = v4i{k2, k2, k2, k2};
    }
    v4i lab0 = {0x10000, 0x10000, 0x10000, 0x10000};
    asm volatile("" : "+v"(lab0));
#pragma unroll
    for (int h = 0; h < NQ; ++h) asm volatile("" : "+v"(cq[h]), "+v"(kq[h]));
    const int64_t lo = (int64_t)chunk_id * a.chunk;
    const int64_t hi = (lo + a.chunk < a.R) ? lo + a.chunk : a.R;
    const int nbat = (int)((hi - lo + 63) >> 6);
    const int64_t bat0 = lo >> 6;
    uint4* crow[NQ];
#pragma unroll
    for (int h = 0; h < NQ; ++h)
        crow[h] = CACHE ? pair_cache + ((int64_t)chunk_id * (a.qpad >> 4) + (t16 + h)) * ((a.chunk + 63) >> 6) * 64 + lane : nullptr;
    uint32_t wcur[4][NMI], wnxt[4][NMI];
    const int ritem = 4 * (lane & 3) + ((lane & 15) >> 2);
    int wi_c[NMC];
#pragma unroll
    for (int c = 0; c < NMC; ++c) wi_c[c] = 2 * c + rwi < a.W ? 2 * c + rwi : a.W - 1;
    const int lwi = F4 ? slot : rwi;
    const int wi_l = lwi < a.LW ? lwi : (a.LW > 0 ? a.LW - 1 : 0);
    auto load_words = [&](int64_t batch, uint32_t (&w)[4][NMI]) {
        const int64_t first = batch * 64;
        if (first + 64 <= (int64_t)a.R) {
            const uint32_t* __restrict__ pc = a.rbits + (first + ritem) * a.W;
            const uint32_t* __restrict__ pl = a.rlab + (first + ritem) * a.LW;
#pragma unroll
            for (int g = 0; g < 4; ++g) {
#pragma unroll
                for (int c = 0; c < NMC; ++c) w[g][c] = pc[g * 16 * a.W + wi_c[c]];
                w[g][NMC] = pl[g * 16 * a.LW + wi_l];
            }
        } else {
#pragma unroll
            for (int g = 0; g < 4; ++g) {
                const int64_t item = first + g * 16 + ritem;
                const int64_t it = item < a.R ? item : (int64_t)a.R - 1;
                const uint32_t ok = item < a.R ? 0xffffffffu : 0u;
#pragma unroll
                for (int c = 0; c < NMC; ++c) w[g][c] = a.rbits[it * a.W + wi_c[c]] & ok;
                w[g][NMC] = a.rlab[it * a.LW + wi_l] & ok;
            }
        }
    };
    auto build = [&](v4i (&At)[NMI], const uint32_t (&w)[NMI]) {
#pragma unroll
        for (int c = 0; c < NMC; ++c) {
            const uint32_t xa = w[c] >> rsh, xb = w[c] >> (rsh + 2);
            At[c][0] = (int)(xa & 0x01010101u);
            At[c][1] = (int)(xa & 0x02020202u);
            At[c][2] = (int)(xb & 0x01010101u);
            At[c][3] = (int)(xb & 0x02020202u);
        }
        if constexpr (F4) {
            At[NMC] = label_item_f4(w[NMC]);
        } else {
            const uint32_t y = w[NMC] >> rsh;
#pragma unroll
            for (int j = 0; j < 4; ++j) At[NMC][j] = (int)(y & (0x01010101u << j));
        }
    };
    uint32_t dmax = 0u;
    load_words(bat0, wcur);
    for (int i = 0; i < nbat; ++i) {
        load_words(bat0 + (i + 1 < nbat ? i + 1 : i), wnxt);
        v4i A[4][NMI];
        uint32_t cw[NQ][4];
        v4i addr_p = {0, 0, 0, 0}, d2_p = {0, 0, 0, 0}, lab_p = {0, 0, 0, 0};
        auto fused = [&](const v4i (&At)[NMI], int h, v4i& addr, v4i& d2, v4i& lab, uint32_t& i0, uint32_t& i1, uint32_t& i2, uint32_t& i3) {
            if constexpr (F4 && CACHE) XMH_W_FUSED_CACHE(XMH_W_MFMA_F4);
            else if constexpr (F4) XMH_W_FUSED_PLAIN(XMH_W_MFMA_F4);
            else if constexpr (CACHE) XMH_W_FUSED_CACHE(XMH_W_MFMA);
            else XMH_W_FUSED_PLAIN(XMH_W_MFMA);
        };
        auto pack = [&](uint32_t& w, const v4i& d, uint32_t i0, uint32_t i1, uint32_t i2, uint32_t i3) {
            uint32_t wb;
            asm volatile("v_or_b32_sdwa %[wa], %[d0], %[i0] dst_sel:BYTE_0 dst_unused:UNUSED_PAD src0_sel:BYTE_0 src1_sel:BYTE_0\n\t"
                         "v_or_b32_sdwa %[wb], %[d1], %[i1] dst_sel:BYTE_1 dst_unused:UNUSED_PAD src0_sel:BYTE_0 src1_sel:BYTE_0\n\t"
                         "v_max3_u32 %[mx], %[d0], %[d1], %[mx]\n\t"
                         "v_or_b32_sdwa %[wa], %[d2], %[i2] dst_sel:BYTE_2 dst_unused:UNUSED_PRESERVE src0_sel:BYTE_0 src1_sel:BYTE_0\n\t"
                         "v_or_b32_sdwa %[wb], %[d3], %[i3] dst_sel:BYTE_3 dst_unused:UNUSED_PRESERVE src0_sel:BYTE_0 src1_sel:BYTE_0\n\t"
                         "v_max3_u32 %[mx], %[d2], %[d3], %[mx]\n\t"
                         "v_or_b32 %[wa], %[wa], %[wb]"
                         : [wa] "=&v"(w), [wb] "=&v"(wb), [mx] "+v"(dmax)
                         : [d0] "v"(d[0]), [d1] "v"(d[1]), [d2] "v"(d[2]), [d3] "v"(d[3]), [i0] "v"(i0), [i1] "v"(i1), [i2] "v"(i2), [i3] "v"(i3));
        };
        auto evaluate = [&](const v4i (&At)[NMI], int h, v4i& addr, v4i& d2, v4i& lab) {
            if constexpr (F4) {
                asm volatile("s_nop 3\n\t" XMH_W_MFMA_F4("lab", "al0", "bl0", "lab0") : [lab] "=&v"(lab) : [al0] "v"(At[2]), [bl0] "v"(bL[h]), [lab0] "v"(lab0));
            } else {
                asm volatile("s_nop 3\n\t" XMH_W_MFMA("lab", "al0", "bl0", "lab0") : [lab] "=&v"(lab) : [al0] "v"(At[2]), [bl0] "v"(bL[h]), [lab0] "v"(lab0));
            }
            if (CACHE) {
                asm volatile("s_nop 3\n\t" XMH_W_MFMA("addr", "a0", "ba0", "cq") XMH_W_MFMA("addr", "a1", "ba1", "addr") XMH_W_MFMA("d2", "a0", "bd0", "kq")
                             XMH_W_MFMA("d2", "a1", "bd1", "d2") "s_nop 7"
                             : [addr] "=&v"(addr), [d2] "=&v"(d2)
                             : [a0] "v"(At[0]), [a1] "v"(At[1]), [ba0] "v"(bA[h][0]), [ba1] "v"(bA[h][1]), [bd0] "v"(bD[h][0]), [bd1] "v"(bD[h][1]), [cq] "v"(cq[h]),
                               [kq] "v"(kq[h]));
            } else {
                asm volatile("s_nop 3\n\t" XMH_W_MFMA("addr", "a0", "ba0", "cq") XMH_W_MFMA("addr", "a1", "ba1", "addr") "s_nop 7"
                             : [addr] "=&v"(addr)
                             : [a0] "v"(At[0]), [a1] "v"(At[1]), [ba0] "v"(bA[h][0]), [ba1] "v"(bA[h][1]), [cq] "v"(cq[h]));
            }
        };
        auto consume = [&](uint32_t& i0, uint32_t& i1, uint32_t& i2, uint32_t& i3, const v4i (&live)[NMI]) {
            asm volatile(XMH_W_MIN("i0", "lp0") XMH_W_MIN("i1", "lp1") XMH_W_MIN("i2", "lp2") XMH_W_MIN("i3", "lp3") XMH_W_ADD("ap0", "i0")
                         XMH_W_ADD("ap1", "i1") XMH_W_ADD("ap2", "i2") XMH_W_ADD("ap3", "i3")
                         : [i0] "=&v"(i0), [i1] "=&v"(i1), [i2] "=&v"(i2), [i3] "=&v"(i3)
                         : [lp0] "v"(lab_p[0]), [lp1] "v"(lab_p[1]), [lp2] "v"(lab_p[2]), [lp3] "v"(lab_p[3]), [ap0] "v"(addr_p[0]), [ap1] "v"(addr_p[1]),
                           [ap2] "v"(addr_p[2]), [ap3] "v"(addr_p[3]), "v"(live[0]), "v"(live[1]), "v"(live[2])
                         : "memory");
        };
        auto group = [&](auto gc) {
            constexpr int G = decltype(gc)::value;
#pragma unroll
            for (int h = 0; h < NQ; ++h) {
                v4i addr, d2 = d2_p, lab;
                if (G == 0 && h == 0) {
                    evaluate(A[G], h, addr, d2, lab);
                } else {
                    uint32_t i0, i1, i2, i3;
                    fused(A[G], h, addr, d2, lab, i0, i1, i2, i3);
                    if (CACHE) pack(cw[(h + NQ - 1) % NQ][h == 0 ? G - 1 : G], d2_p, i0, i1, i2, i3);
                }
                addr_p = addr; d2_p = d2; lab_p = lab;
                if (G > 0 && h == 0) {
                    asm volatile("" ::"v"(A[G > 0 ? G - 1 : 0][0]), "v"(A[G > 0 ? G - 1 : 0][1]), "v"(A[G > 0 ? G - 1 : 0][2]));
                }
            }
        };
        build(A[0], wcur[0]);
        build(A[1], wcur[1]);
        build(A[2], wcur[2]);
        build(A[3], wcur[3]);
        group(std::integral_constant<int, 0>{});
        group(std::integral_constant<int, 1>{});
        group(std::integral_constant<int, 2>{});
        group(std::integral_constant<int, 3>{});
        asm volatile("s_nop 7\n\ts_nop 3" ::: "memory");
        {
            uint32_t i0, i1, i2, i3;
            consume(i0, i1, i2, i3, A[3]);
            if (CACHE) pack(cw[NQ - 1][3], d2_p, i0, i1, i2, i3);
        }
#ifdef XMH_ABL_NOSTORE
        if (CACHE && a.Q < 0) {
#else
        if (CACHE) {
#endif
#pragma unroll
            for (int h = 0; h < NQ; ++h) {
                uint4* dst = crow[h] + (int64_t)i * 64;
                __builtin_nontemporal_store(cw[h][0], &dst->x);
                __builtin_nontemporal_store(cw[h][1], &dst->y);
                __builtin_nontemporal_store(cw[h][2], &dst->z);
                __builtin_nontemporal_store(cw[h][3], &dst->w);
            }
        }
#pragma unroll
        for (int g = 0; g < 4; ++g)
#pragma unroll
            for (int m = 0; m < NMI; ++m) wcur[g][m] = wnxt[g][m];
    }
    const int npad = nbat * 64 - (int)(hi - lo);
    asm volatile("s_waitcnt lgkmcnt(0)" ::: "memory");
    if (npad > 0 && slot == 0) {
#pragma unroll
        for (int h = 0; h < NQ; ++h) {
            if (!valid[h]) continue;
            const int64_t q = (int64_t)(t16 + h) * 16 + ql;
            int dpad = 0;
            for (int w = 0; w < a.W; ++w) dpad += __popc(a.qbits[q * a.W + w]);
            cnt[h * ncell + dpad * 16 + ql] -= (uint32_t)npad << 16;
        }
    }
#pragma unroll
    for (int h = 0; h < NQ; ++h) {
        uint32_t* __restrict__ out = chunk_hist + ((int64_t)chunk_id * a.nb) * a.qpad + (t16 + h) * 16;
        for (int e = lane; e < ncell; e += 64) out[(int64_t)(e >> 4) * a.qpad + (e & 15)] = cnt[h * ncell + e];
    }
    if (CACHE && dmax >= 256u) *ovf = 1u;
}
#undef XMH_W_FUSED_PLAIN
#undef XMH_W_FUSED_CACHE
#undef XMH_W_MFMA_F4
#undef XMH_W_MFMA
#undef XMH_W_MIN
#undef XMH_W_ADD

template <bool CAPPED, int EB, bool HALF = false>
__global__ __launch_bounds__(64) void k_scan_ap_c(ScanArgs a, const uint2* __restrict__ below, const uint2* __restrict__ dpre,
                                                  const uint32_t* __restrict__ cap_ws, float* __restrict__ ap_part,
                                                  const uint32_t* __restrict__ items_total, uint32_t kcap, const uint32_t* __restrict__ skip_if = nullptr,
                                                  const uint32_t* __restrict__ nrel_max = nullptr, int rank_bits = 0) {
    static_assert(!HALF || EB == 8, "the 8 x 8 geometry on one-byte entries");
    constexpr int QW = HALF ? 8 : 128 / EB, LOG_QW = QW == 16 ? 4 : 3, S = 64 / QW, EPW = HALF ? 2 : 32 / EB;
    extern __shared__ __attribute__((aligned(16))) uint32_t lds[];
    int chunk_id, qtile;
    if (!map_block(a, chunk_id, qtile)) return;
    if (items_total && (int64_t)*items_total > kFloatBitsMaxItems) return;
    if (skip_if && *skip_if != 0u) return;
    if (nrel_max && rank_bits > 0 && (uint64_t)(*nrel_max) + 2 < (1ull << (32 - rank_bits))) return;
    const int lane = threadIdx.x & 63;
    const int ql = lane & (QW - 1), slot = lane >> LOG_QW;
    const int q0 = qtile * QW, q = q0 + ql;
    const int ncell = a.nb * QW;
    unsigned long long* cnt = reinterpret_cast<unsigned long long*>(lds);
    {
        const uint2* __restrict__ pb = below + ((int64_t)chunk_id * a.nb) * a.qpad + q0;
        const uint2* __restrict__ pd = dpre + q0;
        auto pack = [](uint2 x, uint2 y) {
            return (unsigned long long)(kF23 + x.x + y.x + 1u) | ((unsigned long long)(kF23 + (0x7fffffu - (x.y + y.y + 1u))) << 32);
        };
        int e = lane;
        for (; e + 7 * 64 < ncell; e += 8 * 64) {
            uint2 x[8], y[8];
#pragma unroll
            for (int j = 0; j < 8; ++j) {
                const int ee = e + j * 64;
                const int64_t at = (int64_t)(ee >> LOG_QW) * a.qpad + (ee & (QW - 1));
                x[j] = pb[at];
                y[j] = pd[at];
            }
#pragma unroll
            for (int j = 0; j < 8; ++j) cnt[e + j * 64] = pack(x[j], y[j]);
        }
        for (; e < ncell; e += 64) {
            const int64_t at = (int64_t)(e >> LOG_QW) * a.qpad + (e & (QW - 1));
            cnt[e] = pack(pb[at], pd[at]);
        }
    }
    const uint32_t cntbase = (uint32_t)(uintptr_t)(__attribute__((address_space(3))) uint32_t*)lds + ql * 8;
    const float capf = CAPPED ? (float)min(cap_ws[q], kcap) : 0.0f;
    const int64_t lo = (int64_t)chunk_id * a.chunk;
    const int64_t hi = (lo + a.chunk < a.R) ? lo + a.chunk : a.R;
    float acc = 0.0f;
    auto credit = [&](unsigned long long old, uint32_t m) {
        const float rank = __uint_as_float((uint32_t)old) - 8388608.0f;
        const float ord = 16777215.0f - __uint_as_float((uint32_t)(old >> 32));
        if (CAPPED) m = ord <= capf ? m : 0u;
#ifdef XMH_ABL_AP_NORCP
        acc = fmaf(ord, __uint_as_float(__float_as_uint(rank) & m), acc);
#else
        acc = fmaf(ord, __uint_as_float(__float_as_uint(__builtin_amdgcn_rcpf(rank)) & m), acc);
#endif
    };
    const uint32_t hoff = HALF ? 8u * (uint32_t)(slot >> 2) : 0u;
    const uint32_t hb0 = hoff, hb1 = hoff + 16u, hd0 = hoff + 1u, hd1 = hoff + 17u;
    auto issue1 = [&](uint32_t w, int j, unsigned long long& old, uint32_t& m) {
        uint32_t d;
        if (HALF) {
            m = (uint32_t)__builtin_amdgcn_sbfe((int)w, j ? hb1 : hb0, 1);
            d = __builtin_amdgcn_ubfe(w, j ? hd1 : hd0, EB - 1);
        } else if (EB == 16) {
            m = (uint32_t)__builtin_amdgcn_sbfe((int)w, j, 1);
            d = __builtin_amdgcn_ubfe(w, j + 1, 11);
        } else {
            m = (uint32_t)__builtin_amdgcn_sbfe((int)w, EB * j, 1);
            d = __builtin_amdgcn_ubfe(w, EB * j + 1, EB - 1);
        }
        uint32_t addr;
        if (QW == 16) asm("v_lshl_add_u32 %0, %1, 7, %2" : "=v"(addr) : "v"(d), "v"(cntbase));
        else asm("v_lshl_add_u32 %0, %1, 6, %2" : "=v"(addr) : "v"(d), "v"(cntbase));
        const unsigned long long inc = 1ull | ((unsigned long long)m << 32);
#ifdef XMH_ABL_AP_NOATOMIC
        old = ((unsigned long long)addr << 3) | inc;
        asm volatile("" : "+v"(old));
#else
        asm volatile("ds_add_rtn_u64 %0, %1, %2" : "=v"(old) : "v"(addr), "v"(inc) : "memory");
#endif
    };
    unsigned long long oldA[8], oldB[8];
    uint32_t mA[8], mB[8];
    constexpr bool kFourBatchIterations = true;
    auto issue = [&](unsigned long long (&old)[8], uint32_t (&m)[8], uint32_t wa, uint32_t wb, uint32_t wc, uint32_t wd) {
        if constexpr (EB == 16) {
            const uint32_t sx = __builtin_amdgcn_alignbit(wb, wa, 24), sy = __builtin_amdgcn_alignbit(wc, wb, 28);
#pragma unroll
            for (int u = 0; u < 8; ++u) issue1(XMH_CACHE12_WORD(u, wa, wb, wc, sx, sy), XMH_CACHE12_BIT(u), old[u], m[u]);
        } else {
#pragma unroll
            for (int u = 0; u < 8; ++u) {
                const int wi = u / EPW;
                issue1(wi == 0 ? wa : (wi == 1 ? wb : (wi == 2 ? wc : wd)), u % EPW, old[u], m[u]);
            }
        }
    };
    auto drain8 = [&](unsigned long long (&old)[8], uint32_t (&m)[8]) {
        asm volatile("s_waitcnt lgkmcnt(8)" : "+v"(old[0]), "+v"(old[1]), "+v"(old[2]), "+v"(old[3]), "+v"(old[4]), "+v"(old[5]), "+v"(old[6]), "+v"(old[7])::"memory");
#pragma unroll
        for (int u = 0; u < 8; ++u) credit(old[u], m[u]);
    };
    auto drain0 = [&](unsigned long long (&old)[8], uint32_t (&m)[8]) {
        asm volatile("s_waitcnt lgkmcnt(0)" : "+v"(old[0]), "+v"(old[1]), "+v"(old[2]), "+v"(old[3]), "+v"(old[4]), "+v"(old[5]), "+v"(old[6]), "+v"(old[7])::"memory");
#pragma unroll
        for (int u = 0; u < 8; ++u) credit(old[u], m[u]);
    };
    const int nbatch = (a.chunk + 63) >> 6;
    const uint4* crow = HALF ? a.pair_cache + ((int64_t)chunk_id * (a.nqt >> 1) + (qtile >> 1)) * nbatch * 64 + (slot & 3) * 16 + (qtile & 1) * 8 + ql
                             : a.pair_cache + ((int64_t)chunk_id * a.nqt + qtile) * nbatch * 64 + lane;
    const int nfull = (int)((hi - lo) >> 6);
    asm volatile("s_waitcnt lgkmcnt(0)" ::: "memory");
    const uint32_t* crow12 = reinterpret_cast<const uint32_t*>(a.pair_cache) + (((int64_t)chunk_id * a.nqt + qtile) * nbatch * 64 + lane) * xmh::kCache12Dwords;
    auto cache_words = [&](int64_t batch) -> uint4 {
        if constexpr (EB == 16) {
            typedef uint32_t u32x3_t __attribute__((ext_vector_type(3)));
            const u32x3_t v = __builtin_nontemporal_load(reinterpret_cast<const u32x3_t*>(crow12 + batch * 64 * xmh::kCache12Dwords));
            return make_uint4(v.x, v.y, v.z, 0u);
        } else {
#ifdef XMH_ABL_AP_PLAIN
            return crow[batch * 64];
#else
            typedef uint32_t u32x4_t __attribute__((ext_vector_type(4)));
            const u32x4_t v = __builtin_nontemporal_load(reinterpret_cast<const u32x4_t*>(crow + batch * 64));
            return make_uint4(v.x, v.y, v.z, v.w);
#endif
        }
    };
    uint4 cw = cache_words(0);
    uint4 nw = cache_words(1 < nbatch ? 1 : 0);
    auto next_words = [&](int bi) {
#ifdef XMH_ABL_AP_NOLOAD
        const uint4 nw2 = make_uint4(0x10203040u + bi + lane, 0x18283848u ^ lane, 0x11223344u + 3 * lane, 0x21314151u + bi);
#else
        const uint4 nw2 = cache_words(bi + 2 < nbatch ? bi + 2 : nbatch - 1);
#endif
        return nw2;
    };
    auto slow_batch = [&](const uint4& w4, int count) {
        const uint32_t sx = EB == 16 ? __builtin_amdgcn_alignbit(w4.y, w4.x, 24) : 0u, sy = EB == 16 ? __builtin_amdgcn_alignbit(w4.z, w4.y, 28) : 0u;
#pragma unroll
        for (int t = 0; t < QW; ++t) {
            if (t * S + slot < count) {
                const uint32_t w = EB == 16 ? XMH_CACHE12_WORD(t, w4.x, w4.y, w4.z, sx, sy) : (t < EPW ? w4.x : (t < 2 * EPW ? w4.y : (t < 3 * EPW ? w4.z : w4.w)));
                const uint32_t bit = EB == 16 ? (uint32_t)XMH_CACHE12_BIT(t) : (HALF ? hoff + 16u * (t % EPW) : (uint32_t)(EB * (t % EPW)));
                const uint32_t m = (uint32_t)__builtin_amdgcn_sbfe((int)w, bit, 1), d = __builtin_amdgcn_ubfe(w, bit + 1u, EB == 16 ? 11 : EB - 1);
                const unsigned long long o = atomicAdd(&cnt[d * QW + ql], 1ull | ((unsigned long long)m << 32));
                credit(o, m);
            }
        }
    };
    if (EB == 8 && !HALF) {
        int bi = 0;
        if (kFourBatchIterations) {
            for (; bi + 3 < nfull; bi += 4) {
                const uint4 n0 = next_words(bi);
                issue(oldA, mA, cw.x, cw.y, 0u, 0u);
                issue(oldB, mB, cw.z, cw.w, 0u, 0u);
                drain8(oldA, mA);
                cw = nw;
                nw = n0;
#pragma unroll
                for (int t = 1; t < 4; ++t) {
                    const uint4 nt = next_words(bi + t);
                    issue(oldA, mA, cw.x, cw.y, 0u, 0u);
                    drain8(oldB, mB);
                    issue(oldB, mB, cw.z, cw.w, 0u, 0u);
                    drain8(oldA, mA);
                    cw = nw;
                    nw = nt;
                }
                drain0(oldB, mB);
            }
        }
        for (; bi + 1 < nfull; bi += 2) {
            const uint4 nw2 = next_words(bi);
            issue(oldA, mA, cw.x, cw.y, 0u, 0u);
            issue(oldB, mB, cw.z, cw.w, 0u, 0u);
            drain8(oldA, mA);
            cw = nw;
            nw = nw2;
            const uint4 nw3 = next_words(bi + 1);
            issue(oldA, mA, cw.x, cw.y, 0u, 0u);
            drain8(oldB, mB);
            issue(oldB, mB, cw.z, cw.w, 0u, 0u);
            drain8(oldA, mA);
            drain0(oldB, mB);
            cw = nw;
            nw = nw3;
        }
        if (bi < nfull) {
            const uint4 nw2 = next_words(bi);
            issue(oldA, mA, cw.x, cw.y, 0u, 0u);
            issue(oldB, mB, cw.z, cw.w, 0u, 0u);
            drain8(oldA, mA);
            drain0(oldB, mB);
            cw = nw;
            nw = nw2;
        }
    } else {
        auto words_at = [&](int b) { return cache_words(b < nbatch ? b : nbatch - 1); };
        auto issue4 = [&](unsigned long long (&old)[8], uint32_t (&m)[8], const uint4& r) { issue(old, m, r.x, r.y, r.z, r.w); };
        uint4 r0 = cw, r1 = nw, r2 = words_at(2), r3 = words_at(3);
        int bi = 0;
        for (; bi + 3 < nfull; bi += 4) {
            issue4(oldA, mA, r0);
            r0 = words_at(bi + 4);
            issue4(oldB, mB, r1);
            r1 = words_at(bi + 5);
            drain8(oldA, mA);
            issue4(oldA, mA, r2);
            r2 = words_at(bi + 6);
            drain8(oldB, mB);
            issue4(oldB, mB, r3);
            r3 = words_at(bi + 7);
            drain8(oldA, mA);
            drain0(oldB, mB);
        }
        const int rem = nfull - bi;
        if (rem >= 2) {
            issue4(oldA, mA, r0);
            issue4(oldB, mB, r1);
            drain8(oldA, mA);
            drain0(oldB, mB);
            if (rem == 3) {
                issue4(oldA, mA, r2);
                drain0(oldA, mA);
            }
        } else if (rem == 1) {
            issue4(oldA, mA, r0);
            drain0(oldA, mA);
        }
        cw = rem == 0 ? r0 : (rem == 1 ? r1 : (rem == 2 ? r2 : r3));
    }
    const int cntb = (int)(hi - lo) - nfull * 64;
    slow_batch(cw, cntb);
#pragma unroll
    for (int o = QW; o < 64; o <<= 1) acc += __shfl_xor(acc, o, 64);
    if (slot == 0) ap_part[(int64_t)chunk_id * a.qpad + q] = acc;
}

#define XMH_AP2_SETA "v113", "v115", "v117", "v119", "v[112:113]", "v[114:115]", "v[116:117]", "v[118:119]"
#define XMH_AP2_SETB "v121", "v123", "v125", "v127", "v[120:121]", "v[122:123]", "v[124:125]", "v[126:127]"
#define XMH_AP2_MFMA(D, A, B, C) "v_mfma_i32_16x16x64_i8 %[" D "], %[" A "], %[" B "], " C "\n\t"
#define XMH_AP2_MFMA_F4(D, A, B, C) "v_mfma_f32_16x16x128_f8f6f4 %[" D "], %[" A "], %[" B "], " C " cbsz:4 blgp:4\n\t"
#define XMH_AP2_MAX(H, L) "v_max_i32 " H ", -1, %[" L "]\n\t"
#define XMH_AP2_ADD(O, A, P) "ds_add_rtn_u64 %[" O "], %[" A "], " P "\n\t"
#define XMH_AP2_FUSED_(LAB, H0, H1, H2, H3, P0, P1, P2, P3)                                                                              \
    "s_nop 3\n\t" LAB("lab", "a1", "q1", "0") XMH_AP2_MAX(H0, "l0") XMH_AP2_MAX(H1, "l1") XMH_AP2_MAX(H2, "l2") XMH_AP2_MAX(H3, "l3")    \
    XMH_AP2_MFMA("addr", "a0", "q0", "%[c0]") XMH_AP2_ADD("o0", "p0", P0) XMH_AP2_ADD("o1", "p1", P1) XMH_AP2_ADD("o2", "p2", P2)       \
    XMH_AP2_ADD("o3", "p3", P3)
#define XMH_AP2_TAIL_(H0, H1, H2, H3, P0, P1, P2, P3)                                                                                     \
    XMH_AP2_MAX(H0, "l0") XMH_AP2_MAX(H1, "l1") XMH_AP2_MAX(H2, "l2") XMH_AP2_MAX(H3, "l3") XMH_AP2_ADD("o0", "p0", P0)                   \
    XMH_AP2_ADD("o1", "p1", P1) XMH_AP2_ADD("o2", "p2", P2) XMH_AP2_ADD("o3", "p3", P3)
#define XMH_AP2_FUSED(...) XMH_AP2_FUSED_(__VA_ARGS__)
#define XMH_AP2_TAIL(...) XMH_AP2_TAIL_(__VA_ARGS__)
template <int NML, int NW, int NQ, bool CAPPED>
__global__ __launch_bounds__(64 * NW) void k_scan_ap_r2(MfmaArgs a, const uint2* __restrict__ below, const uint2* __restrict__ dpre,
                                                        const uint32_t* __restrict__ cap_ws, float* __restrict__ ap_part,
                                                        const uint32_t* __restrict__ items_total, uint32_t kcap) {
    using u64 = unsigned long long;
    static_assert(NML == 1 || NML == 2, "one i8 label tile (at most 64 classes) or one FP4 label tile (65-128 classes)");
    constexpr bool F4 = NML == 2;
    constexpr int NMI = 2;
    extern __shared__ __attribute__((aligned(16))) uint32_t lds[];
    int chunk_id, qtile;
    if (!map_block(a, chunk_id, qtile)) return;
    if (items_total && (int64_t)*items_total > kFloatBitsMaxItems) return;
    const int lane = threadIdx.x & 63, wave = threadIdx.x >> 6;
    const int ql = lane & 15, slot = lane >> 4;
    const int t16 = (qtile * NW + wave) * NQ;
    const int ncell = a.nb * 16;
    u64* cnt = reinterpret_cast<u64*>(lds) + (wave * NQ) * ncell;
    auto pack = [](uint2 x, uint2 y) {
        return (u64)(kF23 + x.x + y.x + 1u) | ((u64)(kF23 + (0x7fffffu - (x.y + y.y + 1u))) << 32);
    };
#pragma unroll
    for (int h = 0; h < NQ; ++h) {
        const uint2* __restrict__ pb = below + ((int64_t)chunk_id * a.nb) * a.qpad + (t16 + h) * 16;
        const uint2* __restrict__ pd = dpre + (t16 + h) * 16;
        u64* c = cnt + h * ncell;
        auto cell = [&](int e) { return e; };
        int e = lane;
        for (; e + 3 * 64 < ncell; e += 4 * 64) {
            uint2 x[4], y[4];
#pragma unroll
            for (int j = 0; j < 4; ++j) {
                const int ee = e + j * 64;
                const int64_t at = (int64_t)(ee >> 4) * a.qpad + (ee & 15);
                x[j] = pb[at];
                y[j] = pd[at];
            }
#pragma unroll
            for (int j = 0; j < 4; ++j) c[cell(e + j * 64)] = pack(x[j], y[j]);
        }
        for (; e < ncell; e += 64) {
            const int64_t at = (int64_t)(e >> 4) * a.qpad + (e & 15);
            c[cell(e)] = pack(pb[at], pd[at]);
        }
    }
    v4i bq[NQ], bl[NQ], cq[NQ];
    float capf[NQ], acc[NQ];
    const int rsh = 4 * (slot & 1), rwi = slot >> 1;
#pragma unroll
    for (int h = 0; h < NQ; ++h) {
        const int64_t q = (int64_t)(t16 + h) * 16 + ql;
        const bool valid = q < a.Q;
        int pcq = 0;
        uint32_t qw = 0u;
        if (valid) {
            for (int w = 0; w < a.W; ++w) pcq += __popc(a.qbits[q * a.W + w]);
            if (rwi < a.W) qw = a.qbits[q * a.W + rwi];
        }
        qw >>= rsh;
        const bool on = valid && rwi < a.W;
#pragma unroll
        for (int j = 0; j < 4; ++j) {
            const uint32_t t = (qw >> j) & 0x01010101u;
            if (j & 1) bq[h][j] = on ? (int)(0x20202020u ^ (t * 0xc0u)) : 0;
            else bq[h][j] = on ? (int)(0x40404040u ^ (t << 7)) : 0;
        }
        if constexpr (F4) {
            bl[h] = label_query_f4(valid && slot < a.LW ? a.qlab[q * a.LW + slot] : 0u, 0xAu);
        } else {
            uint32_t lw = 0u;
            if (valid && rwi < a.LW) lw = a.qlab[q * a.LW + rwi];
            lw >>= rsh;
#pragma unroll
            for (int j = 0; j < 4; ++j) bl[h][j] = (int)(((lw >> j) & 0x01010101u) * 0xffu);
        }
        const int c0 = (int)(uint32_t)(uintptr_t)(__attribute__((address_space(3))) u64*)(cnt + h * ncell) + ql * 8 + (valid ? 128 * pcq : 0);
        cq[h] = v4i{c0, c0, c0, c0};
        asm volatile("" : "+v"(cq[h]));
        capf[h] = CAPPED ? (float)min(cap_ws[q], kcap) : 0.0f;
        acc[h] = 0.0f;
    }
    const int64_t lo = (int64_t)chunk_id * a.chunk;
    const int64_t hi = (lo + a.chunk < a.R) ? lo + a.chunk : a.R;
    const int nbat = (int)((hi - lo + 63) >> 6);
    const int64_t bat0 = lo >> 6;
    uint32_t wcur[4][NMI], wnxt[4][NMI];
    const int ritem = 4 * (lane & 3) + ((lane & 15) >> 2);
    const int wi_c = rwi < a.W ? rwi : a.W - 1;
    const int lwi = F4 ? slot : rwi;
    const int wi_l = lwi < a.LW ? lwi : (a.LW > 0 ? a.LW - 1 : 0);
    auto load_words = [&](int64_t batch, uint32_t (&w)[4][NMI]) {
        const int64_t first = batch * 64;
        if (first + 64 <= (int64_t)a.R) {
            const uint32_t* __restrict__ pc = a.rbits + (first + ritem) * a.W + wi_c;
            const uint32_t* __restrict__ pl = a.rlab + (first + ritem) * a.LW;
#pragma unroll
            for (int g = 0; g < 4; ++g) {
                w[g][0] = pc[g * 16 * a.W];
                w[g][1] = pl[g * 16 * a.LW + wi_l];
            }
        } else {
#pragma unroll
            for (int g = 0; g < 4; ++g) {
                const int64_t item = first + g * 16 + ritem;
                const int64_t it = item < a.R ? item : (int64_t)a.R - 1;
                const uint32_t ok = item < a.R ? 0xffffffffu : 0u;
                w[g][0] = a.rbits[it * a.W + wi_c] & ok;
                w[g][1] = a.rlab[it * a.LW + wi_l] & ok;
            }
        }
    };
    const uint32_t rot_a = (uint32_t)(rsh + 31) & 31u, rot_b = (uint32_t)rsh + 1u;
    auto build = [&](v4i (&At)[NMI], const uint32_t (&w)[NMI]) {
        const uint32_t xa = __builtin_amdgcn_alignbit(w[0], w[0], rot_a), xb = __builtin_amdgcn_alignbit(w[0], w[0], rot_b);
        At[0][0] = (int)(xa & 0x02020202u);
        At[0][1] = (int)(xa & 0x04040404u);
        At[0][2] = (int)(xb & 0x02020202u);
        At[0][3] = (int)(xb & 0x04040404u);
        if constexpr (F4) {
            At[1] = label_item_f4(w[1]);
        } else {
            const uint32_t y = w[1] >> rsh;
#pragma unroll
            for (int j = 0; j < 4; ++j) At[1][j] = (int)(y & (0x01010101u << j));
        }
    };
    auto credit = [&](u64 old, uint32_t m, int h) {
        const float rank = __uint_as_float((uint32_t)old) - 8388608.0f;
        const float ord = 16777215.0f - __uint_as_float((uint32_t)(old >> 32));
        if (CAPPED) m = ord <= capf[h] ? m : 0u;
        acc[h] = fmaf(ord, __uint_as_float(__float_as_uint(__builtin_amdgcn_rcpf(rank)) & m), acc[h]);
    };
    v4i incA01 = {1, 0, 1, 0}, incA23 = {1, 0, 1, 0}, incB01 = {1, 0, 1, 0}, incB23 = {1, 0, 1, 0};
    asm volatile("" : "+{v[112:115]}"(incA01), "+{v[116:119]}"(incA23), "+{v[120:123]}"(incB01), "+{v[124:127]}"(incB23));
    asm volatile("s_waitcnt lgkmcnt(0)" ::: "memory");
    load_words(bat0, wcur);
    for (int i = 0; i < nbat; ++i) {
        load_words(bat0 + (i + 1 < nbat ? i + 1 : i), wnxt);
        v4i A[4][NMI];
        build(A[0], wcur[0]);
        build(A[1], wcur[1]);
        build(A[2], wcur[2]);
        build(A[3], wcur[3]);
        u64 oldA[4], oldB[4];
        v4i addr_p, lab_p;
        auto evaluate = [&](const v4i (&At)[NMI], int h, v4i& addr, v4i& lab) {
            if constexpr (F4)
                asm volatile("s_nop 3\n\t" XMH_AP2_MFMA_F4("lab", "a1", "q1", "0") XMH_AP2_MFMA("addr", "a0", "q0", "%[c0]") "s_nop 7"
                             : [lab] "=&v"(lab), [addr] "=&v"(addr)
                             : [a1] "v"(At[1]), [q1] "v"(bl[h]), [a0] "v"(At[0]), [q0] "v"(bq[h]), [c0] "v"(cq[h]));
            else
                asm volatile("s_nop 3\n\t" XMH_AP2_MFMA("lab", "a1", "q1", "0") XMH_AP2_MFMA("addr", "a0", "q0", "%[c0]") "s_nop 7"
                             : [lab] "=&v"(lab), [addr] "=&v"(addr)
                             : [a1] "v"(At[1]), [q1] "v"(bl[h]), [a0] "v"(At[0]), [q0] "v"(bq[h]), [c0] "v"(cq[h]));
        };
#define XMH_AP2_OUTS(OLD) [lab] "=&v"(lab), [addr] "=&v"(addr), [o0] "=&v"(OLD[0]), [o1] "=&v"(OLD[1]), [o2] "=&v"(OLD[2]), [o3] "=&v"(OLD[3])
#define XMH_AP2_PREV [p0] "v"(addr_p[0]), [p1] "v"(addr_p[1]), [p2] "v"(addr_p[2]), [p3] "v"(addr_p[3]), [l0] "v"(lab_p[0]), [l1] "v"(lab_p[1]), [l2] "v"(lab_p[2]), [l3] "v"(lab_p[3])
        auto fusedA = [&](const v4i (&At)[NMI], int h, v4i& addr, v4i& lab) {
            if constexpr (F4)
                asm volatile(XMH_AP2_FUSED(XMH_AP2_MFMA_F4, XMH_AP2_SETA)
                             : XMH_AP2_OUTS(oldA), "+{v[112:115]}"(incA01), "+{v[116:119]}"(incA23)
                             : [a1] "v"(At[1]), [q1] "v"(bl[h]), [a0] "v"(At[0]), [q0] "v"(bq[h]), [c0] "v"(cq[h]), XMH_AP2_PREV
                             : "memory");
            else
                asm volatile(XMH_AP2_FUSED(XMH_AP2_MFMA, XMH_AP2_SETA)
                             : XMH_AP2_OUTS(oldA), "+{v[112:115]}"(incA01), "+{v[116:119]}"(incA23)
                             : [a1] "v"(At[1]), [q1] "v"(bl[h]), [a0] "v"(At[0]), [q0] "v"(bq[h]), [c0] "v"(cq[h]), XMH_AP2_PREV
                             : "memory");
        };
        auto fusedB = [&](const v4i (&At)[NMI], int h, v4i& addr, v4i& lab) {
            if constexpr (F4)
                asm volatile(XMH_AP2_FUSED(XMH_AP2_MFMA_F4, XMH_AP2_SETB)
                             : XMH_AP2_OUTS(oldB), "+{v[120:123]}"(incB01), "+{v[124:127]}"(incB23)
                             : [a1] "v"(At[1]), [q1] "v"(bl[h]), [a0] "v"(At[0]), [q0] "v"(bq[h]), [c0] "v"(cq[h]), XMH_AP2_PREV
                             : "memory");
            else
                asm volatile(XMH_AP2_FUSED(XMH_AP2_MFMA, XMH_AP2_SETB)
                             : XMH_AP2_OUTS(oldB), "+{v[120:123]}"(incB01), "+{v[124:127]}"(incB23)
                             : [a1] "v"(At[1]), [q1] "v"(bl[h]), [a0] "v"(At[0]), [q0] "v"(bq[h]), [c0] "v"(cq[h]), XMH_AP2_PREV
                             : "memory");
        };
        auto drainA = [&](int h, auto newer) {
            if constexpr (decltype(newer)::value == 4) asm volatile("s_waitcnt lgkmcnt(4)" : "+v"(oldA[0]), "+v"(oldA[1]), "+v"(oldA[2]), "+v"(oldA[3])::"memory");
            else asm volatile("s_waitcnt lgkmcnt(0)" : "+v"(oldA[0]), "+v"(oldA[1]), "+v"(oldA[2]), "+v"(oldA[3])::"memory");
            credit(oldA[0], (uint32_t)incA01[1], h);
            credit(oldA[1], (uint32_t)incA01[3], h);
            credit(oldA[2], (uint32_t)incA23[1], h);
            credit(oldA[3], (uint32_t)incA23[3], h);
        };
        auto drainB = [&](int h, auto newer) {
            if constexpr (decltype(newer)::value == 4) asm volatile("s_waitcnt lgkmcnt(4)" : "+v"(oldB[0]), "+v"(oldB[1]), "+v"(oldB[2]), "+v"(oldB[3])::"memory");
            else asm volatile("s_waitcnt lgkmcnt(0)" : "+v"(oldB[0]), "+v"(oldB[1]), "+v"(oldB[2]), "+v"(oldB[3])::"memory");
            credit(oldB[0], (uint32_t)incB01[1], h);
            credit(oldB[1], (uint32_t)incB01[3], h);
            credit(oldB[2], (uint32_t)incB23[1], h);
            credit(oldB[3], (uint32_t)incB23[3], h);
        };
        using N4 = std::integral_constant<int, 4>;
        using N0 = std::integral_constant<int, 0>;
        auto step = [&](auto pc) {
            constexpr int P = decltype(pc)::value, G = P / NQ, H = P % NQ;
            v4i addr, lab;
            if constexpr (P == 0) evaluate(A[0], 0, addr, lab);
            else if constexpr ((P - 1) & 1) fusedB(A[G], H, addr, lab);
            else fusedA(A[G], H, addr, lab);
            addr_p = addr; lab_p = lab;
            if constexpr (G > 0 && H == 0) {
                asm volatile("" ::"v"(A[G - 1][0]), "v"(A[G - 1][1]));
            }
            if constexpr (P >= 2) {
                if constexpr ((P - 2) & 1) drainB((P - 2) % NQ, N4{});
                else drainA((P - 2) % NQ, N4{});
            }
        };
        auto run = [&](auto self, auto pc) -> void {
            step(pc);
            if constexpr (decltype(pc)::value + 1 < 4 * NQ) self(self, std::integral_constant<int, decltype(pc)::value + 1>{});
        };
        run(run, std::integral_constant<int, 0>{});
        asm volatile("s_nop 7\n\ts_nop 3" ::: "memory");
        {
            constexpr int PL = 4 * NQ - 1;
            static_assert(PL & 1, "the last pair of a batch goes to set B");
            asm volatile(XMH_AP2_TAIL(XMH_AP2_SETB)
                         : [o0] "=&v"(oldB[0]), [o1] "=&v"(oldB[1]), [o2] "=&v"(oldB[2]), [o3] "=&v"(oldB[3]), "+{v[120:123]}"(incB01), "+{v[124:127]}"(incB23)
                         : XMH_AP2_PREV, "v"(A[3][0]), "v"(A[3][1]), "v"(A[3][NMI - 1])
                         : "memory");
            drainA((PL - 1) % NQ, N4{});
            drainB(PL % NQ, N0{});
        }
#pragma unroll
        for (int g = 0; g < 4; ++g)
#pragma unroll
            for (int m = 0; m < NMI; ++m) wcur[g][m] = wnxt[g][m];
    }
#undef XMH_AP2_OUTS
#undef XMH_AP2_PREV
#pragma unroll
    for (int h = 0; h < NQ; ++h) {
        float s = acc[h];
        s += __shfl_xor(s, 16, 64);
        s += __shfl_xor(s, 32, 64);
        if (slot == 0) ap_part[(int64_t)chunk_id * a.qpad + (t16 + h) * 16 + ql] = s;
    }
}


}
```

Baseline: 1770 billion pairs/s.

## Derive distance from counter address and move query offset into ds_add immediate

Restructures the MFMA Hamming histogram kernels so the bucket address MFMA also encodes the distance, with 2*distance in byte 1 of the address. This drops the separate distance MFMA and its query-bias registers (NMQ 3 to 2). The LDS counter table is interleaved across waves and query tiles, so each query's base becomes a compile-time ds_add offset immediate instead of a per-query register. Bit extraction uses a rotate plus masks, and the self-check gains edge cases and a static-LDS check. The aim is fewer MFMAs and fewer VGPRs per item, at the cost of tighter constraints on NW, the 16-bit offset range and the overflow threshold.

Measured after the change: 1817 billion pairs/s (median of 6 runs). 1.03x the previous value.

```diff
diff --git a/clip-based-cross-modal-hash_amd/csrc/xmh_scan.hip b/clip-based-cross-modal-hash_amd/csrc/xmh_scan.hip
--- a/clip-based-cross-modal-hash_amd/csrc/xmh_scan.hip
+++ b/clip-based-cross-modal-hash_amd/csrc/xmh_scan.hip
@@ -413,6 +413,8 @@
         g.lds = nb * (64 / l.S) * 8; g.nqt = (int)p.nqtile * l.S;
     } else if (l.kern == Kern::kHistB) {
         g.nqt = (int)(p.qpad / (16 * kMfmaWaves));
+    } else if (l.kern == Kern::kHistR2 || l.kern == Kern::kHistR2w) {
+        g.lds = r2_lds_bytes(l.S, (int)nb); g.nqt = (int)(p.qpad / (l.NW * l.S * 16));
     } else {
         g.lds = (size_t)l.NW * l.S * nb * 16 * (ap ? 8 : 4); g.nqt = (int)(p.qpad / (l.NW * l.S * 16));
     }
@@ -777,10 +779,22 @@
     std::lock_guard<std::mutex> lock(mu);
     if (state[dev]) return state[dev] == 1;
     state[dev] = 1;
-    const int64_t Q = 200, R = 9000;
+    const int64_t Q = 272, R = 9000;
     bool same = true, ran = true;
+    {
+        const void* const r2_kernels[] = {reinterpret_cast<const void*>(k_scan_hist_r2<1, 4, 4, true>), reinterpret_cast<const void*>(k_scan_hist_r2<1, 4, 4, false>),
+                                          reinterpret_cast<const void*>(k_scan_hist_r2<2, 4, 4, true>), reinterpret_cast<const void*>(k_scan_hist_r2<2, 4, 4, false>),
+                                          reinterpret_cast<const void*>(k_scan_hist_r2w<1, 4, 2, true>), reinterpret_cast<const void*>(k_scan_hist_r2w<1, 4, 2, false>),
+                                          reinterpret_cast<const void*>(k_scan_hist_r2w<2, 4, 2, true>), reinterpret_cast<const void*>(k_scan_hist_r2w<2, 4, 2, false>)};
+        for (const void* k : r2_kernels) {
+            hipFuncAttributes fa;
+            if (hipFuncGetAttributes(&fa, k) != hipSuccess) ran = false;
+            else if (fa.sharedSizeBytes != 0) same = false;
+        }
+    }
     const int cases[6][2] = {{64, 80}, {40, 80}, {16, 80}, {100, 80}, {64, 128}, {100, 128}};
     for (const auto& kc : cases) {
+        if (!ran || !same) break;
         const int K = kc[0], C = kc[1], LW = (C + 31) / 32;
         const int W = (K + 31) / 32;
         std::vector<uint32_t> qb(Q * W), ql(Q * LW), rb(R * W), rl(R * LW);
@@ -807,6 +821,19 @@
             }
             for (int w = 0; w < LW; ++w) ql[1 * LW + w] = rl[2 * LW + w] = rl[5000 * LW + w] = 0xffffffffu;
         }
+        {
+            const int64_t q0 = K <= 64 ? 240 : 112;
+            for (int64_t t = 0; t < 16; ++t) {
+                const int64_t q = q0 + t;
+                ql[q * LW] |= 1u;
+                for (int set = 0; set < 2; ++set)
+                    for (int v = 0; v < 4; ++v) {
+                        const int64_t i = (set ? R - 64 : 128) + 4 * t + v;
+                        for (int w = 0; w < W; ++w) rb[i * W + w] = (v & 2) ? ~qb[q * W + w] & (w == W - 1 ? last : 0xffffffffu) : qb[q * W + w];
+                        for (int w = 0; w < LW; ++w) rl[i * LW + w] = (v & 1) ? 0u : ql[q * LW + w];
+                    }
+            }
+        }
         std::vector<uint32_t> h1, h0;
         std::vector<double> a1, a0;
         std::vector<int32_t> c1, c0;
diff --git a/clip-based-cross-modal-hash_amd/csrc/xmh_scan_mfma.h b/clip-based-cross-modal-hash_amd/csrc/xmh_scan_mfma.h
--- a/clip-based-cross-modal-hash_amd/csrc/xmh_scan_mfma.h
+++ b/clip-based-cross-modal-hash_amd/csrc/xmh_scan_mfma.h
@@ -2,6 +2,7 @@
 #include "xmh_common.h"
 #include "xmh_scan_map.h"
 #include <type_traits>
+#include <utility>
 
 namespace {
 
@@ -53,11 +54,22 @@
     return v4i{(int)(w & 0x11111111u), (int)(w & 0x22222222u), (int)(w & 0x44444444u), (int)((w >> 1) & 0x44444444u)};
 }
 
+constexpr int kR2TableRows = 65, kR2RowBytes = 512;
+__device__ __forceinline__ int r2_cell(int wave, int h, int d, int ql) {
+    return ((h >> 1) * kR2TableRows + d) * (kR2RowBytes / 4) + (h & 1) * 64 + wave * 16 + ql;
+}
+constexpr int r2_imm(int h) { return (h & 1) * 256 + (h >> 1) * (kR2TableRows * kR2RowBytes); }
+constexpr size_t r2_lds_bytes(int nq, int nb) { return (size_t)(((nq + 1) / 2 - 1) * kR2TableRows + nb) * kR2RowBytes; }
+template <typename F, int... I>
+__device__ __forceinline__ void r2_each(F&& f, std::integer_sequence<int, I...>) { (f(std::integral_constant<int, I>{}), ...); }
+
 template <int NML, int NW, int NQ, bool CACHE>
 __device__ __forceinline__ void scan_hist_r2_body(const MfmaArgs& a, uint32_t* __restrict__ chunk_hist, uint4* __restrict__ pair_cache) {
     static_assert(NML == 1 || NML == 2, "one i8 label tile (at most 64 classes) or one FP4 label tile (65-128 classes)");
+    static_assert(NW <= 4, "the register part of a counter address, 64 wave + 4 query, stays below 256: byte 1 of the address is 2 * distance");
+    static_assert(r2_imm(NQ - 1) < 65536, "the offset: immediate of ds_add_u32 has 16 bits");
     constexpr bool F4 = NML == 2;
-    constexpr int NMI = 2, NMQ = 3;
+    constexpr int NMI = 2, NMQ = 2;
     constexpr bool REGS = true;
     extern __shared__ __attribute__((aligned(16))) uint32_t lds[];
     int chunk_id, qtile;
@@ -66,9 +78,10 @@
     const int ql = lane & 15, slot = lane >> 4;
     const int t16 = (qtile * NW + wave) * NQ;
     const int ncell = a.nb * 16;
-    uint32_t* cnt = lds + (wave * NQ) * ncell;
-    for (int e = lane; e < NQ * ncell; e += 64) cnt[e] = 0u;
-    v4i bq[NQ][NMQ], cq[NQ], kqv[REGS ? NQ : 1];
+#pragma unroll
+    for (int h = 0; h < NQ; ++h)
+        for (int e = lane; e < ncell; e += 64) lds[r2_cell(wave, h, e >> 4, e & 15)] = 0u;
+    v4i bq[NQ][NMQ], cq[NQ];
     bool valid[NQ];
     const int rsh = 4 * (slot & 1), rwi = slot >> 1;
 #pragma unroll
@@ -87,35 +100,26 @@
             for (int j = 0; j < 4; ++j) {
                 const uint32_t t = (qw >> j) & 0x01010101u;
                 const bool on = valid[h] && rwi < a.W;
-                if (j & 1) {
-                    bq[h][0][j] = on ? (int)(0x20202020u ^ (t * 0xc0u)) : 0;
-                    bq[h][1][j] = on ? (int)(0x01010101u ^ (t * 0xfeu)) : 0;
-                } else {
-                    bq[h][0][j] = on ? (int)(0x40404040u ^ (t << 7)) : 0;
-                    bq[h][1][j] = on ? (int)(0x02020202u ^ (t * 0xfcu)) : 0;
-                }
+                const uint32_t pos = 0x40u >> j, flip = pos ^ ((0x100u - pos) & 0xffu);
+                bq[h][0][j] = on ? (int)((0x01010101u * pos) ^ (t * flip)) : 0;
             }
             if constexpr (F4) {
-                bq[h][2] = label_query_f4(valid[h] && slot < a.LW ? a.qlab[q * a.LW + slot] : 0u, 0x2u);
+                bq[h][1] = label_query_f4(valid[h] && slot < a.LW ? a.qlab[q * a.LW + slot] : 0u, 0x2u);
             } else {
                 uint32_t lw = 0u;
                 if (valid[h] && rwi < a.LW) lw = a.qlab[q * a.LW + rwi];
                 lw >>= rsh;
 #pragma unroll
-                for (int j = 0; j < 4; ++j) bq[h][2][j] = (int)((lw >> j) & 0x01010101u);
-            }
-            const int k2 = 2 * pcq;
-            kqv[h] = v4i{k2, k2, k2, k2};
-        }
-        const int c0 = (int)(uint32_t)(uintptr_t)(__attribute__((address_space(3))) uint32_t*)(cnt + h * ncell) + ql * 4 + (valid[h] ? 64 * pcq : 0);
+                for (int j = 0; j < 4; ++j) bq[h][1][j] = (int)((lw >> j) & 0x01010101u);
+            }
+        }
+        const int c0 = 64 * wave + ql * 4 + (valid[h] ? kR2RowBytes * pcq : 0);
         cq[h] = v4i{c0, c0, c0, c0};
     }
     v4i lab0 = {0x10000, 0x10000, 0x10000, 0x10000};
     asm volatile("" : "+v"(lab0));
 #pragma unroll
     for (int h = 0; h < NQ; ++h) asm volatile("" : "+v"(cq[h]));
-#pragma unroll
-    for (int h = 0; h < (REGS ? NQ : 1); ++h) asm volatile("" : "+v"(kqv[h]));
     const int64_t lo = (int64_t)chunk_id * a.chunk;
     const int64_t hi = (lo + a.chunk < a.R) ? lo + a.chunk : a.R;
     const int nbat = (int)((hi - lo + 63) >> 6);
@@ -150,12 +154,11 @@
             }
         }
     };
+    const uint32_t rot = rsh ? 1u : 29u;
     auto build = [&](v4i (&At)[NMI], const uint32_t (&w)[NMI]) {
-        const uint32_t xa = w[0] >> rsh, xb = w[0] >> (rsh + 2);
-        At[0][0] = (int)(xa & 0x01010101u);
-        At[0][1] = (int)(xa & 0x02020202u);
-        At[0][2] = (int)(xb & 0x01010101u);
-        At[0][3] = (int)(xb & 0x02020202u);
+        const uint32_t x = __builtin_rotateright32(w[0], rot);
+#pragma unroll
+        for (int j = 0; j < 4; ++j) At[0][j] = (int)(x & (0x08080808u << j));
         if constexpr (F4) {
             At[1] = label_item_f4(w[1]);
         } else {
@@ -178,7 +181,7 @@
         v4i A[REGS ? 4 : 2][NMI];
 #endif
         uint32_t cw[NQ][4];
-        v4i addr_p, d2_p, lab_p;
+        v4i addr_p, lab_p;
 #ifndef XMH_R2_NOPS
 #define XMH_R2_NOPS 0
 #endif
@@ -212,10 +215,13 @@
 #undef XMH_VMIN
 #define XMH_VMIN "v_and_b32 "
 #endif
+#if defined(XMH_ABL_NOMFMA) && !defined(XMH_ABL_NOADD)
+#define XMH_ABL_NOADD
+#endif
 #ifdef XMH_ABL_NOADD
-#define XMH_ADD(A, D) "s_nop 0\n\t"
+#define XMH_ADD(A, D, O) "s_nop 0\n\t"
 #else
-#define XMH_ADD(A, D) "ds_add_u32 " A ", " D "\n\t"
+#define XMH_ADD(A, D, O) "ds_add_u32 " A ", " D " offset:" O "\n\t"
 #endif
 #ifdef XMH_ABL_NOMFMA
 #define XMH_MFMA(D, A, B, C) "s_nop 0\n\t"
@@ -224,76 +230,71 @@
 #define XMH_MFMA(D, A, B, C) "v_mfma_i32_16x16x64_i8 " D ", " A ", " B ", " C "\n\t"
 #define XMH_MFMA_F4(D, A, B, C) "v_mfma_f32_16x16x128_f8f6f4 " D ", " A ", " B ", " C " cbsz:4 blgp:4\n\t"
 #endif
-#define XMH_SDWA(J) "dst_sel:BYTE_" #J " dst_unused:UNUSED_PRESERVE src0_sel:BYTE_0 src1_sel:BYTE_0\n\t"
+#define XMH_SDWA(J) "dst_sel:BYTE_" #J " dst_unused:UNUSED_PRESERVE src0_sel:BYTE_1 src1_sel:BYTE_0\n\t"
 #define XMH_R2_FUSED_CACHE(LAB)                                                                                                                   \
-    asm volatile(XMH_R2_OPEN LAB("%0", "%8", "%9", "%10")                                                                                         \
-                 XMH_VMIN "%4, 0x10001, %24\n\t" XMH_VMIN "%5, 0x10001, %25\n\t" XMH_VMIN "%6, 0x10001, %26\n\t" XMH_VMIN "%7, 0x10001, %27\n\t" \
-                 "v_or_b32_sdwa %3, %16, %4 dst_sel:BYTE_0 dst_unused:UNUSED_PAD src0_sel:BYTE_0 src1_sel:BYTE_0\n\t"                            \
-                 XMH_ADD("%20", "%4")                                                                                                             \
-                 XMH_MFMA("%1", "%11", "%12", "%13")                                                                                              \
-                 "v_or_b32_sdwa %3, %17, %5 " XMH_SDWA(1) XMH_ADD("%21", "%5") "v_or_b32_sdwa %3, %18, %6 " XMH_SDWA(2)                           \
-                 XMH_MFMA("%2", "%11", "%14", "%15")                                                                                              \
-                 XMH_ADD("%22", "%6") "v_or_b32_sdwa %3, %19, %7 " XMH_SDWA(3) XMH_ADD("%23", "%7")                                               \
-                 : "=&v"(lab), "=&v"(addr), "=&v"(d2), "=&v"(w), "=&v"(i0), "=&v"(i1), "=&v"(i2), "=&v"(i3)                                        \
-                 : "v"(At[1]), "v"(bq[h][2]), "v"(lab0), "v"(At[0]), "v"(bq[h][0]), "v"(cq[h]), "v"(bq[h][1]), "v"(kqv[REGS ? h : 0]),             \
-                   "v"(d2_p[0]), "v"(d2_p[1]), "v"(d2_p[2]), "v"(d2_p[3]), "v"(addr_p[0]), "v"(addr_p[1]), "v"(addr_p[2]), "v"(addr_p[3]),         \
-                   "v"(lab_p[0]), "v"(lab_p[1]), "v"(lab_p[2]), "v"(lab_p[3])                                                                      \
+    asm volatile(XMH_R2_OPEN LAB("%0", "%7", "%8", "%9")                                                                                          \
+                 XMH_VMIN "%3, 0x10001, %17\n\t" XMH_VMIN "%4, 0x10001, %18\n\t" XMH_VMIN "%5, 0x10001, %19\n\t" XMH_VMIN "%6, 0x10001, %20\n\t" \
+                 "v_or_b32_sdwa %2, %13, %3 dst_sel:BYTE_0 dst_unused:UNUSED_PAD src0_sel:BYTE_1 src1_sel:BYTE_0\n\t"                            \
+                 XMH_ADD("%13", "%3", "%21")                                                                                                      \
+                 XMH_MFMA("%1", "%10", "%11", "%12")                                                                                              \
+                 "v_or_b32_sdwa %2, %14, %4 " XMH_SDWA(1) XMH_ADD("%14", "%4", "%21") "v_or_b32_sdwa %2, %15, %5 " XMH_SDWA(2)                    \
+                 XMH_ADD("%15", "%5", "%21") "v_or_b32_sdwa %2, %16, %6 " XMH_SDWA(3) XMH_ADD("%16", "%6", "%21")                                 \
+                 : "=&v"(lab), "=&v"(addr), "=&v"(w), "=&v"(i0), "=&v"(i1), "=&v"(i2), "=&v"(i3)                                                   \
+                 : "v"(At[1]), "v"(bql), "v"(lab0), "v"(At[0]), "v"(bqa), "v"(cqh),                                                                \
+                   "v"(addr_p[0]), "v"(addr_p[1]), "v"(addr_p[2]), "v"(addr_p[3]), "v"(lab_p[0]), "v"(lab_p[1]), "v"(lab_p[2]), "v"(lab_p[3]),     \
+                   "n"(r2_imm(HP))                                                                                                                 \
                  : "memory")
 #define XMH_R2_FUSED_PLAIN(LAB)                                                                                                                   \
     asm volatile(XMH_R2_OPEN LAB("%0", "%6", "%7", "%8")                                                                                          \
                  XMH_VMIN "%2, 0x10001, %16\n\t" XMH_VMIN "%3, 0x10001, %17\n\t" XMH_VMIN "%4, 0x10001, %18\n\t" XMH_VMIN "%5, 0x10001, %19\n\t" \
                  XMH_MFMA("%1", "%9", "%10", "%11")                                                                                               \
-                 XMH_ADD("%12", "%2") XMH_ADD("%13", "%3") XMH_ADD("%14", "%4") XMH_ADD("%15", "%5")                                              \
+                 XMH_ADD("%12", "%2", "%20") XMH_ADD("%13", "%3", "%20") XMH_ADD("%14", "%4", "%20") XMH_ADD("%15", "%5", "%20")                  \
                  : "=&v"(lab), "=&v"(addr), "=&v"(i0), "=&v"(i1), "=&v"(i2), "=&v"(i3)                                                             \
-                 : "v"(At[1]), "v"(bq[h][2]), "v"(lab0), "v"(At[0]), "v"(bq[h][0]), "v"(cq[h]),                                                    \
-                   "v"(addr_p[0]), "v"(addr_p[1]), "v"(addr_p[2]), "v"(addr_p[3]), "v"(lab_p[0]), "v"(lab_p[1]), "v"(lab_p[2]), "v"(lab_p[3])      \
+                 : "v"(At[1]), "v"(bql), "v"(lab0), "v"(At[0]), "v"(bqa), "v"(cqh),                                                                \
+                   "v"(addr_p[0]), "v"(addr_p[1]), "v"(addr_p[2]), "v"(addr_p[3]), "v"(lab_p[0]), "v"(lab_p[1]), "v"(lab_p[2]), "v"(lab_p[3]),     \
+                   "n"(r2_imm(HP))                                                                                                                 \
                  : "memory")
-#define XMH_R2_EVAL_CACHE(LAB)                                                                                                                    \
-    asm volatile(XMH_R2_OPEN LAB("%0", "%3", "%4", "%5") XMH_MFMA("%1", "%6", "%7", "%8") XMH_MFMA("%2", "%6", "%9", "%10") XMH_R2_EVAL_CLOSE     \
-                 : "=&v"(lab), "=&v"(addr), "=&v"(d2)                                                                                             \
-                 : "v"(At[1]), "v"(bq[h][2]), "v"(lab0), "v"(At[0]), "v"(bq[h][0]), "v"(cq[h]), "v"(bq[h][1]), "v"(kqv[REGS ? h : 0]))
-#define XMH_R2_EVAL_PLAIN(LAB)                                                                                                                    \
+#define XMH_R2_EVAL(LAB)                                                                                                                          \
     asm volatile(XMH_R2_OPEN LAB("%0", "%2", "%3", "%4") XMH_MFMA("%1", "%5", "%6", "%7") XMH_R2_EVAL_CLOSE                                       \
                  : "=&v"(lab), "=&v"(addr)                                                                                                        \
-                 : "v"(At[1]), "v"(bq[h][2]), "v"(lab0), "v"(At[0]), "v"(bq[h][0]), "v"(cq[h]))
-        auto fused = [&](const v4i (&At)[NMI], int h, v4i& addr, v4i& d2, v4i& lab, uint32_t& w) {
+                 : "v"(At[1]), "v"(bql), "v"(lab0), "v"(At[0]), "v"(bqa), "v"(cqh))
+        auto fused = [](auto hc, const v4i (&At)[NMI], const v4i& bqa, const v4i& bql, const v4i& cqh, const v4i& lab0, const v4i& addr_p, const v4i& lab_p,
+                        v4i& addr, v4i& lab, uint32_t& w) {
+            constexpr int HP = (decltype(hc)::value + NQ - 1) % NQ;
             uint32_t i0, i1, i2, i3;
             if constexpr (F4 && CACHE) XMH_R2_FUSED_CACHE(XMH_MFMA_F4);
             else if constexpr (F4) XMH_R2_FUSED_PLAIN(XMH_MFMA_F4);
             else if constexpr (CACHE) XMH_R2_FUSED_CACHE(XMH_MFMA);
             else XMH_R2_FUSED_PLAIN(XMH_MFMA);
         };
-        auto evaluate = [&](const v4i (&At)[NMI], int h, v4i& addr, v4i& d2, v4i& lab) {
-            if constexpr (F4 && CACHE) XMH_R2_EVAL_CACHE(XMH_MFMA_F4);
-            else if constexpr (F4) XMH_R2_EVAL_PLAIN(XMH_MFMA_F4);
-            else if constexpr (CACHE) XMH_R2_EVAL_CACHE(XMH_MFMA);
-            else XMH_R2_EVAL_PLAIN(XMH_MFMA);
+        auto evaluate = [](const v4i (&At)[NMI], const v4i& bqa, const v4i& bql, const v4i& cqh, const v4i& lab0, v4i& addr, v4i& lab) {
+            if constexpr (F4) XMH_R2_EVAL(XMH_MFMA_F4);
+            else XMH_R2_EVAL(XMH_MFMA);
         };
         auto consume = [&](uint32_t& w, const v4i (&live)[NMI]) {
             uint32_t i0, i1, i2, i3;
             if (CACHE) {
                 asm volatile(
                     XMH_VMIN "%1, 0x10001, %5\n\t" XMH_VMIN "%2, 0x10001, %6\n\t" XMH_VMIN "%3, 0x10001, %7\n\t" XMH_VMIN "%4, 0x10001, %8\n\t"
-                    "v_or_b32_sdwa %0, %9, %1 dst_sel:BYTE_0 dst_unused:UNUSED_PAD src0_sel:BYTE_0 src1_sel:BYTE_0\n\t"
-                    XMH_ADD("%13", "%1")
-                    "v_or_b32_sdwa %0, %10, %2 " XMH_SDWA(1) XMH_ADD("%14", "%2") "v_or_b32_sdwa %0, %11, %3 " XMH_SDWA(2)
-                    XMH_ADD("%15", "%3") "v_or_b32_sdwa %0, %12, %4 " XMH_SDWA(3) XMH_ADD("%16", "%4")
+                    "v_or_b32_sdwa %0, %9, %1 dst_sel:BYTE_0 dst_unused:UNUSED_PAD src0_sel:BYTE_1 src1_sel:BYTE_0\n\t"
+                    XMH_ADD("%9", "%1", "%16")
+                    "v_or_b32_sdwa %0, %10, %2 " XMH_SDWA(1) XMH_ADD("%10", "%2", "%16") "v_or_b32_sdwa %0, %11, %3 " XMH_SDWA(2)
+                    XMH_ADD("%11", "%3", "%16") "v_or_b32_sdwa %0, %12, %4 " XMH_SDWA(3) XMH_ADD("%12", "%4", "%16")
                     : "=&v"(w), "=&v"(i0), "=&v"(i1), "=&v"(i2), "=&v"(i3)
-                    : "v"(lab_p[0]), "v"(lab_p[1]), "v"(lab_p[2]), "v"(lab_p[3]), "v"(d2_p[0]), "v"(d2_p[1]), "v"(d2_p[2]), "v"(d2_p[3]), "v"(addr_p[0]),
-                      "v"(addr_p[1]), "v"(addr_p[2]), "v"(addr_p[3]), "v"(live[0]), "v"(live[1]), "v"(live[NMI - 1])
+                    : "v"(lab_p[0]), "v"(lab_p[1]), "v"(lab_p[2]), "v"(lab_p[3]), "v"(addr_p[0]), "v"(addr_p[1]), "v"(addr_p[2]), "v"(addr_p[3]),
+                      "v"(live[0]), "v"(live[1]), "v"(live[NMI - 1]), "n"(r2_imm(NQ - 1))
                     : "memory");
             } else {
                 asm volatile(
                     XMH_VMIN "%0, 0x10001, %4\n\t" XMH_VMIN "%1, 0x10001, %5\n\t" XMH_VMIN "%2, 0x10001, %6\n\t" XMH_VMIN "%3, 0x10001, %7\n\t"
-                    XMH_ADD("%8", "%0") XMH_ADD("%9", "%1") XMH_ADD("%10", "%2") XMH_ADD("%11", "%3")
+                    XMH_ADD("%8", "%0", "%15") XMH_ADD("%9", "%1", "%15") XMH_ADD("%10", "%2", "%15") XMH_ADD("%11", "%3", "%15")
                     : "=&v"(i0), "=&v"(i1), "=&v"(i2), "=&v"(i3)
                     : "v"(lab_p[0]), "v"(lab_p[1]), "v"(lab_p[2]), "v"(lab_p[3]), "v"(addr_p[0]), "v"(addr_p[1]), "v"(addr_p[2]), "v"(addr_p[3]), "v"(live[0]),
-                      "v"(live[1]), "v"(live[NMI - 1])
+                      "v"(live[1]), "v"(live[NMI - 1]), "n"(r2_imm(NQ - 1))
                     : "memory");
             }
         };
-#undef XMH_R2_EVAL_PLAIN
-#undef XMH_R2_EVAL_CACHE
+#undef XMH_R2_EVAL
 #undef XMH_R2_FUSED_PLAIN
 #undef XMH_R2_FUSED_CACHE
 #undef XMH_SDWA
@@ -303,17 +304,17 @@
         auto group = [&](auto gc) {
             constexpr int G = decltype(gc)::value;
             constexpr int SET = REGS ? G : (G & 1);
-#pragma unroll
-            for (int h = 0; h < NQ; ++h) {
-                v4i addr, d2, lab;
-                if (G == 0 && h == 0) evaluate(A[SET], h, addr, d2, lab);
-                else fused(A[SET], h, addr, d2, lab, cw[(h + NQ - 1) % NQ][h == 0 ? G - 1 : G]);
-                addr_p = addr; d2_p = d2; lab_p = lab;
+            r2_each([&](auto hc) {
+                constexpr int h = decltype(hc)::value;
+                v4i addr, lab;
+                if constexpr (G == 0 && h == 0) evaluate(A[SET], bq[h][0], bq[h][1], cq[h], lab0, addr, lab);
+                else fused(hc, A[SET], bq[h][0], bq[h][1], cq[h], lab0, addr_p, lab_p, addr, lab, cw[(h + NQ - 1) % NQ][h == 0 ? G - 1 : G]);
+                addr_p = addr; lab_p = lab;
                 if (REGS && G > 0 && h == 0) {
                     if constexpr (NMI == 2) asm volatile("" ::"v"(A[REGS ? G - 1 : 0][0]), "v"(A[REGS ? G - 1 : 0][1]));
                     else asm volatile("" ::"v"(A[REGS ? G - 1 : 0][0]), "v"(A[REGS ? G - 1 : 0][1]), "v"(A[REGS ? G - 1 : 0][NMI - 1]));
                 }
-            }
+            }, std::make_integer_sequence<int, NQ>{});
         };
 #ifdef XMH_ABL_NOBUILD
         if (i == 0) {
@@ -359,13 +360,13 @@
             const int64_t q = (int64_t)(t16 + h) * 16 + ql;
             int dpad = 0;
             for (int w = 0; w < a.W; ++w) dpad += __popc(a.qbits[q * a.W + w]);
-            cnt[h * ncell + dpad * 16 + ql] -= (uint32_t)npad << 16;
+            lds[r2_cell(wave, h, dpad, ql)] -= (uint32_t)npad << 16;
         }
     }
 #pragma unroll
     for (int h = 0; h < NQ; ++h) {
         uint32_t* __restrict__ out = chunk_hist + ((int64_t)chunk_id * a.nb) * a.qpad + (t16 + h) * 16;
-        for (int e = lane; e < ncell; e += 64) out[(int64_t)(e >> 4) * a.qpad + (e & 15)] = cnt[h * ncell + e];
+        for (int e = lane; e < ncell; e += 64) out[(int64_t)(e >> 4) * a.qpad + (e & 15)] = lds[r2_cell(wave, h, e >> 4, e & 15)];
     }
 }
 
@@ -399,32 +400,22 @@
 #define XMH_W_MFMA(D, A, B, C) "v_mfma_i32_16x16x64_i8 %[" D "], %[" A "], %[" B "], %[" C "]\n\t"
 #define XMH_W_MFMA_F4(D, A, B, C) "v_mfma_f32_16x16x128_f8f6f4 %[" D "], %[" A "], %[" B "], %[" C "] cbsz:4 blgp:4\n\t"
 #define XMH_W_MIN(I, L) "v_min_u32 %[" I "], 0x10001, %[" L "]\n\t"
-#define XMH_W_ADD(A, D) "ds_add_u32 %[" A "], %[" D "]\n\t"
-#define XMH_W_FUSED_CACHE(LAB) \
-    asm volatile("s_nop 3\n\t" LAB("lab", "al0", "bl0", "lab0") XMH_W_MIN("i0", "lp0") XMH_W_MIN("i1", "lp1") XMH_W_MIN("i2", "lp2")                \
-                 XMH_W_MIN("i3", "lp3") XMH_W_ADD("ap0", "i0") XMH_W_MFMA("addr", "a0", "ba0", "cq") XMH_W_ADD("ap1", "i1")                         \
-                 XMH_W_MFMA("addr", "a1", "ba1", "addr") XMH_W_ADD("ap2", "i2") XMH_W_MFMA("d2", "a0", "bd0", "kq") XMH_W_ADD("ap3", "i3")          \
-                 XMH_W_MFMA("d2", "a1", "bd1", "d2")                                                                                                \
-                 : [lab] "=&v"(lab), [addr] "=&v"(addr), [d2] "=&v"(d2), [i0] "=&v"(i0), [i1] "=&v"(i1), [i2] "=&v"(i2), [i3] "=&v"(i3)             \
-                 : [a0] "v"(At[0]), [a1] "v"(At[1]), [al0] "v"(At[2]), [ba0] "v"(bA[h][0]), [ba1] "v"(bA[h][1]), [bd0] "v"(bD[h][0]),               \
-                   [bd1] "v"(bD[h][1]), [bl0] "v"(bL[h]), [lab0] "v"(lab0), [cq] "v"(cq[h]), [kq] "v"(kq[h]), [lp0] "v"(lab_p[0]),                  \
-                   [lp1] "v"(lab_p[1]), [lp2] "v"(lab_p[2]), [lp3] "v"(lab_p[3]), [ap0] "v"(addr_p[0]), [ap1] "v"(addr_p[1]), [ap2] "v"(addr_p[2]), \
-                   [ap3] "v"(addr_p[3])                                                                                                             \
-                 : "memory")
-#define XMH_W_FUSED_PLAIN(LAB) \
+#define XMH_W_ADD(A, D) "ds_add_u32 %[" A "], %[" D "] offset:%[off]\n\t"
+#define XMH_W_FUSED(LAB) \
     asm volatile("s_nop 3\n\t" LAB("lab", "al0", "bl0", "lab0") XMH_W_MIN("i0", "lp0") XMH_W_MIN("i1", "lp1") XMH_W_MIN("i2", "lp2")                 \
                  XMH_W_MIN("i3", "lp3") XMH_W_ADD("ap0", "i0") XMH_W_ADD("ap1", "i1") XMH_W_MFMA("addr", "a0", "ba0", "cq") XMH_W_ADD("ap2", "i2")   \
                  XMH_W_ADD("ap3", "i3") XMH_W_MFMA("addr", "a1", "ba1", "addr")                                                                      \
                  : [lab] "=&v"(lab), [addr] "=&v"(addr), [i0] "=&v"(i0), [i1] "=&v"(i1), [i2] "=&v"(i2), [i3] "=&v"(i3)                              \
-                 : [a0] "v"(At[0]), [a1] "v"(At[1]), [al0] "v"(At[2]), [ba0] "v"(bA[h][0]), [ba1] "v"(bA[h][1]), [bl0] "v"(bL[h]), [lab0] "v"(lab0), \
-                   [cq] "v"(cq[h]), [lp0] "v"(lab_p[0]), [lp1] "v"(lab_p[1]), [lp2] "v"(lab_p[2]), [lp3] "v"(lab_p[3]), [ap0] "v"(addr_p[0]),        \
-                   [ap1] "v"(addr_p[1]), [ap2] "v"(addr_p[2]), [ap3] "v"(addr_p[3])                                                                  \
+                 : [a0] "v"(At[0]), [a1] "v"(At[1]), [al0] "v"(At[2]), [ba0] "v"(bAh[0]), [ba1] "v"(bAh[1]), [bl0] "v"(bLh), [lab0] "v"(lab0),       \
+                   [cq] "v"(cqh), [lp0] "v"(lab_p[0]), [lp1] "v"(lab_p[1]), [lp2] "v"(lab_p[2]), [lp3] "v"(lab_p[3]), [ap0] "v"(addr_p[0]),        \
+                   [ap1] "v"(addr_p[1]), [ap2] "v"(addr_p[2]), [ap3] "v"(addr_p[3]), [off] "n"(r2_imm(HP))                                           \
                  : "memory")
 template <int NML, int NW, int NQ, bool CACHE>
 __global__ __launch_bounds__(64 * NW) void k_scan_hist_r2w(MfmaArgs a, uint32_t* __restrict__ chunk_hist, uint4* __restrict__ pair_cache,
                                                            uint32_t* __restrict__ ovf) {
     static_assert(NML == 1 || NML == 2, "one i8 label tile (at most 64 classes) or one FP4 label tile (65-128 classes)");
     constexpr bool F4 = NML == 2;
+    static_assert(NW <= 4 && NQ <= 2, "one table of 129 rows: the register part of an address, 64 wave + 4 query, stays below 256, the immediate is 256 h");
     constexpr int NMC = 2, NMI = NMC + 1;
     extern __shared__ __attribute__((aligned(16))) uint32_t lds[];
     int chunk_id, qtile;
@@ -433,10 +424,11 @@
     const int ql = lane & 15, slot = lane >> 4;
     const int t16 = (qtile * NW + wave) * NQ;
     const int ncell = a.nb * 16;
-    uint32_t* cnt = lds + (wave * NQ) * ncell;
-    for (int e = lane; e < NQ * ncell; e += 64) cnt[e] = 0u;
+#pragma unroll
+    for (int h = 0; h < NQ; ++h)
+        for (int e = lane; e < ncell; e += 64) lds[r2_cell(wave, h, e >> 4, e & 15)] = 0u;
     const int rsh = 4 * (slot & 1), rwi = slot >> 1;
-    v4i bA[NQ][NMC], bD[NQ][NMC], bL[NQ], cq[NQ], kq[NQ];
+    v4i bA[NQ][NMC], bL[NQ], cq[NQ];
     bool valid[NQ];
 #pragma unroll
     for (int h = 0; h < NQ; ++h) {
@@ -453,13 +445,8 @@
 #pragma unroll
             for (int j = 0; j < 4; ++j) {
                 const uint32_t t = (qw >> j) & 0x01010101u;
-                if (j & 1) {
-                    bA[h][c][j] = on ? (int)(0x20202020u ^ (t * 0xc0u)) : 0;
-                    bD[h][c][j] = on ? (int)(0x01010101u ^ (t * 0xfeu)) : 0;
-                } else {
-                    bA[h][c][j] = on ? (int)(0x40404040u ^ (t << 7)) : 0;
-                    bD[h][c][j] = on ? (int)(0x02020202u ^ (t * 0xfcu)) : 0;
-                }
+                const uint32_t pos = 0x40u >> j, flip = pos ^ ((0x100u - pos) & 0xffu);
+                bA[h][c][j] = on ? (int)((0x01010101u * pos) ^ (t * flip)) : 0;
             }
         }
         if constexpr (F4) {
@@ -471,15 +458,13 @@
 #pragma unroll
             for (int j = 0; j < 4; ++j) bL[h][j] = (int)((lw >> j) & 0x01010101u);
         }
-        const int c0 = (int)(uint32_t)(uintptr_t)(__attribute__((address_space(3))) uint32_t*)(cnt + h * ncell) + ql * 4 + (valid[h] ? 64 * pcq : 0);
-        const int k2 = valid[h] ? 2 * pcq : 0;
+        const int c0 = 64 * wave + ql * 4 + (valid[h] ? kR2RowBytes * pcq : 0);
         cq[h] = v4i{c0, c0, c0, c0};
-        kq[h] = v4i{k2, k2, k2, k2};
     }
     v4i lab0 = {0x10000, 0x10000, 0x10000, 0x10000};
     asm volatile("" : "+v"(lab0));
 #pragma unroll
-    for (int h = 0; h < NQ; ++h) asm volatile("" : "+v"(cq[h]), "+v"(kq[h]));
+    for (int h = 0; h < NQ; ++h) asm volatile("" : "+v"(cq[h]));
     const int64_t lo = (int64_t)chunk_id * a.chunk;
     const int64_t hi = (lo + a.chunk < a.R) ? lo + a.chunk : a.R;
     const int nbat = (int)((hi - lo + 63) >> 6);
@@ -518,14 +503,13 @@
             }
         }
     };
+    const uint32_t rot = rsh ? 1u : 29u;
     auto build = [&](v4i (&At)[NMI], const uint32_t (&w)[NMI]) {
 #pragma unroll
         for (int c = 0; c < NMC; ++c) {
-            const uint32_t xa = w[c] >> rsh, xb = w[c] >> (rsh + 2);
-            At[c][0] = (int)(xa & 0x01010101u);
-            At[c][1] = (int)(xa & 0x02020202u);
-            At[c][2] = (int)(xb & 0x01010101u);
-            At[c][3] = (int)(xb & 0x02020202u);
+            const uint32_t x = __builtin_rotateright32(w[c], rot);
+#pragma unroll
+            for (int j = 0; j < 4; ++j) At[c][j] = (int)(x & (0x08080808u << j));
         }
         if constexpr (F4) {
             At[NMC] = label_item_f4(w[NMC]);
@@ -541,68 +525,60 @@
         load_words(bat0 + (i + 1 < nbat ? i + 1 : i), wnxt);
         v4i A[4][NMI];
         uint32_t cw[NQ][4];
-        v4i addr_p = {0, 0, 0, 0}, d2_p = {0, 0, 0, 0}, lab_p = {0, 0, 0, 0};
-        auto fused = [&](const v4i (&At)[NMI], int h, v4i& addr, v4i& d2, v4i& lab, uint32_t& i0, uint32_t& i1, uint32_t& i2, uint32_t& i3) {
-            if constexpr (F4 && CACHE) XMH_W_FUSED_CACHE(XMH_W_MFMA_F4);
-            else if constexpr (F4) XMH_W_FUSED_PLAIN(XMH_W_MFMA_F4);
-            else if constexpr (CACHE) XMH_W_FUSED_CACHE(XMH_W_MFMA);
-            else XMH_W_FUSED_PLAIN(XMH_W_MFMA);
+        v4i addr_p = {0, 0, 0, 0}, lab_p = {0, 0, 0, 0};
+        auto fused = [](auto hc, const v4i (&At)[NMI], const v4i (&bAh)[NMC], const v4i& bLh, const v4i& cqh, const v4i& lab0, const v4i& addr_p, const v4i& lab_p,
+                        v4i& addr, v4i& lab, uint32_t& i0, uint32_t& i1, uint32_t& i2, uint32_t& i3) {
+            constexpr int HP = (decltype(hc)::value + NQ - 1) % NQ;
+            if constexpr (F4) XMH_W_FUSED(XMH_W_MFMA_F4);
+            else XMH_W_FUSED(XMH_W_MFMA);
         };
         auto pack = [&](uint32_t& w, const v4i& d, uint32_t i0, uint32_t i1, uint32_t i2, uint32_t i3) {
             uint32_t wb;
-            asm volatile("v_or_b32_sdwa %[wa], %[d0], %[i0] dst_sel:BYTE_0 dst_unused:UNUSED_PAD src0_sel:BYTE_0 src1_sel:BYTE_0\n\t"
-                         "v_or_b32_sdwa %[wb], %[d1], %[i1] dst_sel:BYTE_1 dst_unused:UNUSED_PAD src0_sel:BYTE_0 src1_sel:BYTE_0\n\t"
+            asm volatile("v_or_b32_sdwa %[wa], %[d0], %[i0] dst_sel:BYTE_0 dst_unused:UNUSED_PAD src0_sel:BYTE_1 src1_sel:BYTE_0\n\t"
+                         "v_or_b32_sdwa %[wb], %[d1], %[i1] dst_sel:BYTE_1 dst_unused:UNUSED_PAD src0_sel:BYTE_1 src1_sel:BYTE_0\n\t"
                          "v_max3_u32 %[mx], %[d0], %[d1], %[mx]\n\t"
-                         "v_or_b32_sdwa %[wa], %[d2], %[i2] dst_sel:BYTE_2 dst_unused:UNUSED_PRESERVE src0_sel:BYTE_0 src1_sel:BYTE_0\n\t"
-                         "v_or_b32_sdwa %[wb], %[d3], %[i3] dst_sel:BYTE_3 dst_unused:UNUSED_PRESERVE src0_sel:BYTE_0 src1_sel:BYTE_0\n\t"
+                         "v_or_b32_sdwa %[wa], %[d2], %[i2] dst_sel:BYTE_2 dst_unused:UNUSED_PRESERVE src0_sel:BYTE_1 src1_sel:BYTE_0\n\t"
+                         "v_or_b32_sdwa %[wb], %[d3], %[i3] dst_sel:BYTE_3 dst_unused:UNUSED_PRESERVE src0_sel:BYTE_1 src1_sel:BYTE_0\n\t"
                          "v_max3_u32 %[mx], %[d2], %[d3], %[mx]\n\t"
                          "v_or_b32 %[wa], %[wa], %[wb]"
                          : [wa] "=&v"(w), [wb] "=&v"(wb), [mx] "+v"(dmax)
                          : [d0] "v"(d[0]), [d1] "v"(d[1]), [d2] "v"(d[2]), [d3] "v"(d[3]), [i0] "v"(i0), [i1] "v"(i1), [i2] "v"(i2), [i3] "v"(i3));
         };
-        auto evaluate = [&](const v4i (&At)[NMI], int h, v4i& addr, v4i& d2, v4i& lab) {
+        auto evaluate = [&](const v4i (&At)[NMI], int h, v4i& addr, v4i& lab) {
             if constexpr (F4) {
                 asm volatile("s_nop 3\n\t" XMH_W_MFMA_F4("lab", "al0", "bl0", "lab0") : [lab] "=&v"(lab) : [al0] "v"(At[2]), [bl0] "v"(bL[h]), [lab0] "v"(lab0));
             } else {
                 asm volatile("s_nop 3\n\t" XMH_W_MFMA("lab", "al0", "bl0", "lab0") : [lab] "=&v"(lab) : [al0] "v"(At[2]), [bl0] "v"(bL[h]), [lab0] "v"(lab0));
             }
-            if (CACHE) {
-                asm volatile("s_nop 3\n\t" XMH_W_MFMA("addr", "a0", "ba0", "cq") XMH_W_MFMA("addr", "a1", "ba1", "addr") XMH_W_MFMA("d2", "a0", "bd0", "kq")
-                             XMH_W_MFMA("d2", "a1", "bd1", "d2") "s_nop 7"
-                             : [addr] "=&v"(addr), [d2] "=&v"(d2)
-                             : [a0] "v"(At[0]), [a1] "v"(At[1]), [ba0] "v"(bA[h][0]), [ba1] "v"(bA[h][1]), [bd0] "v"(bD[h][0]), [bd1] "v"(bD[h][1]), [cq] "v"(cq[h]),
-                               [kq] "v"(kq[h]));
-            } else {
-                asm volatile("s_nop 3\n\t" XMH_W_MFMA("addr", "a0", "ba0", "cq") XMH_W_MFMA("addr", "a1", "ba1", "addr") "s_nop 7"
-                             : [addr] "=&v"(addr)
-                             : [a0] "v"(At[0]), [a1] "v"(At[1]), [ba0] "v"(bA[h][0]), [ba1] "v"(bA[h][1]), [cq] "v"(cq[h]));
-            }
+            asm volatile("s_nop 3\n\t" XMH_W_MFMA("addr", "a0", "ba0", "cq") XMH_W_MFMA("addr", "a1", "ba1", "addr") "s_nop 7"
+                         : [addr] "=&v"(addr)
+                         : [a0] "v"(At[0]), [a1] "v"(At[1]), [ba0] "v"(bA[h][0]), [ba1] "v"(bA[h][1]), [cq] "v"(cq[h]));
         };
         auto consume = [&](uint32_t& i0, uint32_t& i1, uint32_t& i2, uint32_t& i3, const v4i (&live)[NMI]) {
             asm volatile(XMH_W_MIN("i0", "lp0") XMH_W_MIN("i1", "lp1") XMH_W_MIN("i2", "lp2") XMH_W_MIN("i3", "lp3") XMH_W_ADD("ap0", "i0")
                          XMH_W_ADD("ap1", "i1") XMH_W_ADD("ap2", "i2") XMH_W_ADD("ap3", "i3")
                          : [i0] "=&v"(i0), [i1] "=&v"(i1), [i2] "=&v"(i2), [i3] "=&v"(i3)
                          : [lp0] "v"(lab_p[0]), [lp1] "v"(lab_p[1]), [lp2] "v"(lab_p[2]), [lp3] "v"(lab_p[3]), [ap0] "v"(addr_p[0]), [ap1] "v"(addr_p[1]),
-                           [ap2] "v"(addr_p[2]), [ap3] "v"(addr_p[3]), "v"(live[0]), "v"(live[1]), "v"(live[2])
+                           [ap2] "v"(addr_p[2]), [ap3] "v"(addr_p[3]), "v"(live[0]), "v"(live[1]), "v"(live[2]), [off] "n"(r2_imm(NQ - 1))
                          : "memory");
         };
         auto group = [&](auto gc) {
             constexpr int G = decltype(gc)::value;
-#pragma unroll
-            for (int h = 0; h < NQ; ++h) {
-                v4i addr, d2 = d2_p, lab;
-                if (G == 0 && h == 0) {
-                    evaluate(A[G], h, addr, d2, lab);
+            r2_each([&](auto hc) {
+                constexpr int h = decltype(hc)::value;
+                v4i addr, lab;
+                if constexpr (G == 0 && h == 0) {
+                    evaluate(A[G], h, addr, lab);
                 } else {
                     uint32_t i0, i1, i2, i3;
-                    fused(A[G], h, addr, d2, lab, i0, i1, i2, i3);
-                    if (CACHE) pack(cw[(h + NQ - 1) % NQ][h == 0 ? G - 1 : G], d2_p, i0, i1, i2, i3);
+                    fused(hc, A[G], bA[h], bL[h], cq[h], lab0, addr_p, lab_p, addr, lab, i0, i1, i2, i3);
+                    if (CACHE) pack(cw[(h + NQ - 1) % NQ][h == 0 ? G - 1 : G], addr_p, i0, i1, i2, i3);
                 }
-                addr_p = addr; d2_p = d2; lab_p = lab;
+                addr_p = addr; lab_p = lab;
                 if (G > 0 && h == 0) {
                     asm volatile("" ::"v"(A[G > 0 ? G - 1 : 0][0]), "v"(A[G > 0 ? G - 1 : 0][1]), "v"(A[G > 0 ? G - 1 : 0][2]));
                 }
-            }
+            }, std::make_integer_sequence<int, NQ>{});
         };
         build(A[0], wcur[0]);
         build(A[1], wcur[1]);
@@ -616,7 +592,7 @@
         {
             uint32_t i0, i1, i2, i3;
             consume(i0, i1, i2, i3, A[3]);
-            if (CACHE) pack(cw[NQ - 1][3], d2_p, i0, i1, i2, i3);
+            if (CACHE) pack(cw[NQ - 1][3], addr_p, i0, i1, i2, i3);
         }
 #ifdef XMH_ABL_NOSTORE
         if (CACHE && a.Q < 0) {
@@ -646,18 +622,17 @@
             const int64_t q = (int64_t)(t16 + h) * 16 + ql;
             int dpad = 0;
             for (int w = 0; w < a.W; ++w) dpad += __popc(a.qbits[q * a.W + w]);
-            cnt[h * ncell + dpad * 16 + ql] -= (uint32_t)npad << 16;
+            lds[r2_cell(wave, h, dpad, ql)] -= (uint32_t)npad << 16;
         }
     }
 #pragma unroll
     for (int h = 0; h < NQ; ++h) {
         uint32_t* __restrict__ out = chunk_hist + ((int64_t)chunk_id * a.nb) * a.qpad + (t16 + h) * 16;
-        for (int e = lane; e < ncell; e += 64) out[(int64_t)(e >> 4) * a.qpad + (e & 15)] = cnt[h * ncell + e];
-    }
-    if (CACHE && dmax >= 256u) *ovf = 1u;
+        for (int e = lane; e < ncell; e += 64) out[(int64_t)(e >> 4) * a.qpad + (e & 15)] = lds[r2_cell(wave, h, e >> 4, e & 15)];
+    }
+    if (CACHE && dmax >= 65536u) *ovf = 1u;
 }
-#undef XMH_W_FUSED_PLAIN
-#undef XMH_W_FUSED_CACHE
+#undef XMH_W_FUSED
 #undef XMH_W_MFMA_F4
 #undef XMH_W_MFMA
 #undef XMH_W_MIN
```
